# StephenNG59/ICP-symm

Hardware: AMD Instinct MI355X
Metric: icp_iterations_per_sec (higher is better)
Workload: dtype f32

## Files before the change

### icp-symm_amd/csrc/engine.cpp

```cpp
#include "engine_internal.h"
#include "robust_loss.h"
#include <limits>

void read_switches(Switches &w)
{
    auto flag = [](const char *n) { return std::getenv(n) != nullptr; };
    auto num = [](const char *n, long def) { const char *e = std::getenv(n); return e ? std::atol(e) : def; };
    auto tri = [](const char *n) { const char *e = std::getenv(n); return e ? (e[0] == '1' ? 1 : 0) : -1; };
    w.allow_any_arch = flag("SYMMICP_ALLOW_ANY_ARCH");
    w.debug_host = flag("SYMMICP_DEBUG_HOST");
    w.debug_counters = flag("SYMMICP_DEBUG_COUNTERS");
    if (const char *e = std::getenv("SYMMICP_DEBUG_TRACE")) w.debug_trace = e;
    if (const char *e = std::getenv("SYMMICP_GRID_PPC")) w.grid_ppc = std::atof(e);
    w.grid_maxlevel = (int)num("SYMMICP_GRID_MAXLEVEL", kMortonBits);
    w.grid_level = (int)num("SYMMICP_GRID_LEVEL", -1);
    if (const char *e = std::getenv("SYMMICP_FIRST_PASS")) w.first_pass = (e[0] == 'p') ? 1 : 0;
    w.oct_leaf = (int)num("SYMMICP_OCT_LEAF", 0);
    if (const char *e = std::getenv("SYMMICP_PACKET_ORDER")) w.packet_order = e[0] != '0';
    if (const char *e = std::getenv("SYMMICP_PACKET_JUMP")) w.packet_jump = (float)std::atof(e);
    w.packet_key_bits = (int)num("SYMMICP_PACKET_KEY_BITS", 16);
    w.packet_chunk = (uint32_t)num("SYMMICP_PACKET_CHUNK", 0);
    w.packet_lds_pad = (uint32_t)num("SYMMICP_PACKET_LDS_PAD", 0);
    w.packet_waves = (uint32_t)num("SYMMICP_PACKET_WAVES", 0);
    w.packet_front_cap = (uint32_t)num("SYMMICP_PACKET_FRONT_CAP", 0);
    if (const char *e = std::getenv("SYMMICP_HOOD_FRAC")) w.hood_frac = std::atof(e);
    w.no_hood = flag("SYMMICP_NO_NEIGHBOURHOOD");
    w.no_cert = flag("SYMMICP_NO_CERT");
    w.walk_full_grid = flag("SYMMICP_WALK_FULL_GRID");
    { const char *e = std::getenv("SYMMICP_HOST_LOOP"); w.host_loop = e && e[0] == '1'; }
    w.no_loop_stragglers = flag("SYMMICP_NO_LOOP_STRAGGLERS");
    w.force_comm = flag("SYMMICP_FORCE_COMM");
    if (const char *e = std::getenv("SYMMICP_PACKET_COST_KEY")) w.packet_cost_key = e[0] != '0';
    w.budget_walk = tri("SYMMICP_BUDGET_WALK");
    w.optimistic = tri("SYMMICP_OPTIMISTIC");
    w.compact = tri("SYMMICP_COMPACT");
    w.pass_blocks = (int)num("SYMMICP_PASS_BLOCKS", 2048);
    w.id_blocks = (int)num("SYMMICP_ID_BLOCKS", 2048);
    w.acc_blocks = (int)num("SYMMICP_ACC_BLOCKS", 512);
    w.fused_blocks = (int)num("SYMMICP_FUSED_BLOCKS", 512);
    w.compact_blocks = (int)num("SYMMICP_COMPACT_BLOCKS", 1280);
    w.feature_nn_splits = (int)num("SYMMICP_FEATURE_NN_SPLITS", 0);
    w.feature_nn_queries = (int)num("SYMMICP_FEATURE_NN_QUERIES", 0);
    w.tune.wave_mode_max = (uint32_t)num("SYMMICP_WAVE_MODE_MAX", 20000);
    w.tune.cells_chunk = (uint32_t)num("SYMMICP_CELLS_CHUNK", 16);
    w.tune.cells_queries = (uint32_t)num("SYMMICP_CELLS_QUERIES", 0);
    w.tune.walk_budget = (uint32_t)num("SYMMICP_WALK_BUDGET", 160);
}

void arena_begin(Arena &a, size_t want)
{
    a.off = 0;
    if (a.cap >= want) return;
    if (a.base) hipFree(a.base);
    a.base = nullptr; a.cap = 0;
    const size_t cap = want + want / 4;
    if (hipMalloc((void **)&a.base, cap) == hipSuccess) a.cap = cap;
    else (void)hipGetLastError();
}


extern "C" {

int symmicp_version(void) { return 100; }

void symmicp_config_default(symmicp_config *cfg)
{
    if (!cfg) return;
    std::memset(cfg, 0, sizeof(*cfg));
    cfg->struct_size = (int32_t)sizeof(*cfg);
    cfg->device = -1;
    cfg->mode = SYMMICP_MODE_QUIRKS;
    cfg->corr = SYMMICP_CORR_IDENTITY;
    cfg->apply = SYMMICP_APPLY_DEFAULT;
    cfg->max_iters = 10;
    cfg->diff_threshold = 1.0f;
    cfg->max_corr_dist = 0.f;
    cfg->fixed_iters = 0;
    cfg->sort_source = 1;
    cfg->verbose = 0;
    cfg->min_normal_dot = -2.0f;
    cfg->eps_rotation = 0.f;
    cfg->eps_translation = 0.f;
}

static int check_cfg(const symmicp_config *cfg)
{
    if (!cfg || cfg->struct_size != (int32_t)sizeof(symmicp_config)) return SYMMICP_ERR_ARG;
    if (!mode_known(cfg->mode)) return SYMMICP_ERR_ARG;
    if (cfg->corr < SYMMICP_CORR_IDENTITY || cfg->corr > SYMMICP_CORR_TREE) return SYMMICP_ERR_ARG;
    if (cfg->apply < SYMMICP_APPLY_DEFAULT || cfg->apply > SYMMICP_APPLY_CUMULATIVE) return SYMMICP_ERR_ARG;
    if (cfg->max_iters < 0) return SYMMICP_ERR_ARG;
    return SYMMICP_OK;
}

int symmicp_create(const symmicp_config *cfg, symmicp_ctx **out)
{
    if (!out) return SYMMICP_ERR_ARG;
    *out = nullptr;
// ... 417 lines not shown
    HIP_TRY(c, kt.alloc_temp(c->arena, n));
    HIP_TRY(c, vt.alloc_temp(c->arena, n));
    HIP_TRY(c, ws.alloc_temp(c->arena, wse));
    launch_bbox(cl.x, cl.y, cl.z, n, bbox.p, c->stream);
    uint32_t hb[6];
    HIP_TRY(c, hipMemcpyAsync(hb, bbox.p, sizeof(hb), hipMemcpyDeviceToHost, c->stream));
    HIP_TRY(c, hipStreamSynchronize(c->stream));
    float lo[3], hi[3];
    for (int k = 0; k < 3; k++) { lo[k] = ord2f(hb[k]); hi[k] = ord2f(hb[3 + k]); }
    float emax = 0.f;
    for (int k = 0; k < 3; k++) {
        if (!std::isfinite(lo[k]) || !std::isfinite(hi[k])) return fail(c, SYMMICP_ERR_ARG, "cloud has non-finite coordinates");
        emax = std::fmax(emax, hi[k] - lo[k]);
    }
    if (!(emax > 0.f)) emax = 1.f;
    const float h0 = emax * 1.00001f / (float)(1 << kMortonBits);
    launch_morton(cl.x, cl.y, cl.z, n, lo[0], lo[1], lo[2], 1.0f / h0, keys.p, vals.p, c->stream);
    radix_sort_pairs(keys.p, vals.p, kt.p, vt.p, n, 3 * kMortonBits, ws.p, wse, c->stream);
    HIP_TRY(c, hipStreamSynchronize(c->stream));
    HIP_TRY(c, hipGetLastError());
    for (int k = 0; k < 3; k++) origin[k] = lo[k];
    *h0_out = h0;
    return SYMMICP_OK;
}

static int build_octree(symmicp_ctx *c, const uint32_t *keys, const float4 *tq, uint32_t n, uint32_t leaf_max, float4 **onodes_out, TargetIndex *ix)
{
    constexpr int NL = kMortonBits + 1;
    DevBuf<uint32_t> nid;
    DevBuf<uint32_t> scan_ws, first;
    float4 *nodes = nullptr;
    HIP_TRY(c, nid.alloc_temp(c->arena, (size_t)NL * n));
    HIP_TRY(c, scan_ws.alloc_temp(c->arena, (size_t)n / 2048 + 2));
    for (int l = 0; l < NL; l++) {
        launch_oct_flags(keys, n, l, nid.p + (size_t)l * n, c->stream);
        launch_exclusive_scan(nid.p + (size_t)l * n, n, scan_ws.p, c->stream);
    }
    uint32_t last_excl[NL], kl[2] = {0, 0};
    for (int l = 0; l < NL; l++)
        HIP_TRY(c, hipMemcpyAsync(&last_excl[l], nid.p + (size_t)l * n + (n - 1), sizeof(uint32_t), hipMemcpyDeviceToHost, c->stream));
    if (n >= 2) HIP_TRY(c, hipMemcpyAsync(kl, keys + (n - 2), 2 * sizeof(uint32_t), hipMemcpyDeviceToHost, c->stream));
    HIP_TRY(c, hipStreamSynchronize(c->stream));
    uint32_t cnt[NL];
    size_t total = 0;
    for (int l = 0; l < NL; l++) {
        const int shift = 3 * (kMortonBits - l);
        const bool last_starts = (n == 1) || (shift < 30 && (kl[1] >> shift) != (kl[0] >> shift));
        cnt[l] = last_excl[l] + (last_starts ? 1u : 0u);
        ix->olevel_off[l] = (uint32_t)total;
        total += cnt[l];
    }
    ix->olevel_off[NL] = (uint32_t)total;
    for (int l = 0; l < NL; l++)
        if (cnt[l] > kOctCfMask) return fail(c, SYMMICP_ERR_SIZE, "octree level exceeds 2^28 nodes (target cloud too large for SYMMICP_CORR_TREE)");
    HIP_TRY(c, first.alloc_temp(c->arena, total + 1));
    HIP_TRY(c, keep_alloc(c, (void **)&nodes, sizeof(float4) * 2 * total));
    for (int l = 0; l < NL; l++)
        launch_oct_first(keys, n, l, nid.p + (size_t)l * n, first.p + ix->olevel_off[l], c->stream);
    for (int l = NL - 1; l >= 0; l--) {
        const bool bottom = (l == NL - 1);
        launch_oct_nodes(l, tq, n, first.p + ix->olevel_off[l], cnt[l], bottom ? nullptr : nid.p + (size_t)(l + 1) * n,
                         bottom ? 0u : cnt[l + 1], bottom ? nullptr : nodes + 2 * (size_t)ix->olevel_off[l + 1],
                         nodes + 2 * (size_t)ix->olevel_off[l], leaf_max, c->stream);
    }
    HIP_TRY(c, hipStreamSynchronize(c->stream));
    HIP_TRY(c, hipGetLastError());
    *onodes_out = nodes;
    ix->onodes = *onodes_out;
    return SYMMICP_OK;
}

static int build_index(symmicp_ctx *c, const CloudSoA &cl, uint32_t n, bool want_grid, float4 *tq, float4 *tn,
                       float4 **boxes_out, uint2 **cells_out, TargetIndex *ix_out, int32_t *glevel_out, int32_t *nlevels_out,
                       float4 **onodes_out = nullptr, uint32_t **ctop_out = nullptr, IndexNotes *notes = nullptr)
{
    DevBuf<uint32_t> order, keys;
    float origin[3], h0;
    int st = morton_order(c, cl, n, order, &keys, origin, &h0);
    if (st != SYMMICP_OK) return st;
    if (notes) { *notes = IndexNotes{}; for (int k = 0; k < 3; k++) notes->origin[k] = origin[k]; notes->h0 = h0; }
    launch_gather_f4(cl.x, cl.y, cl.z, cl.nx, cl.ny, cl.nz, order.p, n, tq, tn, c->stream);
    TargetIndex ix{};
    ix.tq = tq; ix.tn = tn; ix.n = n;
    int glevel = 0;
    if (want_grid) {
        DevBuf<uint32_t> hist;
        HIP_TRY(c, hist.alloc_temp(c->arena, 16));
        launch_level_hist(keys.p, n, hist.p, c->stream);
        uint32_t hh[16];
        HIP_TRY(c, hipMemcpyAsync(hh, hist.p, sizeof(hh), hipMemcpyDeviceToHost, c->stream));
        HIP_TRY(c, hipStreamSynchronize(c->stream));
        if (notes) std::memcpy(notes->hist, hh, sizeof(hh));
        const double ppc = c->sw.grid_ppc;
        int lcap = c->sw.grid_maxlevel;
        if (lcap > kMortonBits) lcap = kMortonBits;
        glevel = 1;
        double occ = 1.0;
        for (int l = 1; l <= lcap; l++) {
            occ += (double)hh[l];
            if ((double)n / occ >= ppc) glevel = l;
        }
        if (c->sw.grid_level >= 0) glevel = c->sw.grid_level;
        if (glevel > lcap) glevel = lcap;
        if (glevel < 0) glevel = 0;
        {
            double occ_l[kMortonBits + 1];
            double o = 1.0;
            occ_l[0] = 1.0;
            for (int l = 1; l <= kMortonBits; l++) { o += (double)hh[l]; occ_l[l] = o; }
            const int lg = glevel >= 2 ? glevel - 1 : 1;
            const double growth = occ_l[lg] / occ_l[lg - 1];
            c->target_surface_like = growth < 5.5;
            if (c->sw.first_pass >= 0) c->target_surface_like = c->sw.first_pass == 1;
        }
    }
    ix.glevel = glevel;
    if (glevel > 0) {
        const int ltop = glevel > 3 ? glevel - 3 : 0;
        const size_t ntop = (size_t)1 << (3 * ltop);
        DevBuf<uint32_t> nid_top, scan_ws;
        HIP_TRY(c, nid_top.alloc_temp(c->arena, n));
        HIP_TRY(c, scan_ws.alloc_temp(c->arena, (size_t)n / 2048 + 2));
        launch_oct_flags(keys.p, n, ltop, nid_top.p, c->stream);
        launch_exclusive_scan(nid_top.p, n, scan_ws.p, c->stream);
        uint32_t last_excl = 0, kl[2] = {0, 0};
        HIP_TRY(c, hipMemcpyAsync(&last_excl, nid_top.p + (n - 1), sizeof(uint32_t), hipMemcpyDeviceToHost, c->stream));
        if (n >= 2) HIP_TRY(c, hipMemcpyAsync(kl, keys.p + (n - 2), 2 * sizeof(uint32_t), hipMemcpyDeviceToHost, c->stream));
        HIP_TRY(c, hipStreamSynchronize(c->stream));
        const int tshift = 3 * (kMortonBits - ltop);
        const bool last_starts = (n == 1) || (tshift < 30 && (kl[1] >> tshift) != (kl[0] >> tshift));
        const size_t nblocks = (size_t)last_excl + (last_starts ? 1 : 0);
        if (notes) { notes->nblocks = (uint32_t)nblocks; notes->ctop_len = (uint32_t)ntop; }
        HIP_TRY(c, keep_alloc(c, (void **)ctop_out, sizeof(uint32_t) * ntop));
        HIP_TRY(c, hipMemsetAsync(*ctop_out, 0xFF, sizeof(uint32_t) * ntop, c->stream));
        HIP_TRY(c, keep_alloc(c, (void **)cells_out, sizeof(uint2) * nblocks * 512));
        HIP_TRY(c, hipMemsetAsync(*cells_out, 0, sizeof(uint2) * nblocks * 512, c->stream));
        launch_cell_table(keys.p, n, glevel, nid_top.p, *ctop_out, *cells_out, c->stream);
        HIP_TRY(c, hipStreamSynchronize(c->stream));
        ix.ctop = *ctop_out;
        ix.cells = *cells_out;
        ix.gdim = 1 << glevel;
        ix.ox = origin[0]; ix.oy = origin[1]; ix.oz = origin[2];
        ix.h = h0 * (float)(1 << (kMortonBits - glevel));
        ix.inv_h = (1.0f / h0) / (float)(1 << (kMortonBits - glevel));
    }
    uint32_t cnt[kMaxTreeLevels], pad[kMaxTreeLevels];
    int nl = 0;
    uint32_t m = (n + kLeaf - 1) / kLeaf;
    size_t total = 0;
    while (true) {
        cnt[nl] = m;
        pad[nl] = (m <= (uint32_t)kFan) ? m : ((m + kFan - 1) / kFan) * kFan;
        ix.level_off[nl] = (uint32_t)total;
        total += pad[nl];
        nl++;
        if (m <= (uint32_t)kFan) break;
        m = pad[nl - 1] / kFan;
        if (nl >= kMaxTreeLevels) return fail(c, SYMMICP_ERR_SIZE, "tree too deep");
    }
    ix.top = nl - 1;
    ix.ntop = cnt[nl - 1];
    HIP_TRY(c, keep_alloc(c, (void **)boxes_out, sizeof(float4) * 2 * total));
    float4 *boxes = *boxes_out;
    launch_leaf_boxes(tq, n, boxes + 2 * (size_t)ix.level_off[0], pad[0], c->stream);
    for (int l = 1; l < nl; l++)
        launch_node_boxes(boxes + 2 * (size_t)ix.level_off[l - 1], pad[l - 1], boxes + 2 * (size_t)ix.level_off[l], pad[l], c->stream);
    ix.boxes = boxes;
    HIP_TRY(c, hipStreamSynchronize(c->stream));
    HIP_TRY(c, hipGetLastError());
    if (onodes_out) {
        uint32_t leaf_max = c->target_surface_like ? 24u : 8u;
        if (c->sw.oct_leaf > 0) leaf_max = (uint32_t)c->sw.oct_leaf;
        if (notes) notes->leaf_max = leaf_max;
        st = build_octree(c, keys.p, tq, n, leaf_max, onodes_out, &ix);
        if (st != SYMMICP_OK) return st;
    }
    *ix_out = ix;
    if (glevel_out) *glevel_out = glevel;
    if (nlevels_out) *nlevels_out = nl;
    return SYMMICP_OK;
}

int symmicp_set_target(symmicp_ctx *c, const float *xyz, size_t xr, size_t xc, const float *nrm, size_t nr, size_t nc, size_t n)
{
    if (!c) return SYMMICP_ERR_ARG;
    if (!xyz || !nrm) return fail(c, SYMMICP_ERR_ARG, "null target cloud (myicp.cpp:102 assert)");
    if (n == 0 || n > 0x7fffffffull) return fail(c, SYMMICP_ERR_SIZE, "target size out of range");
    HIP_TRY(c, hipSetDevice(c->device));
    const double t0 = now_s();
    free_target(c);
    c->begun = false;
    {
        const size_t want = n * 160 + ((size_t)16 << 20);
        if (c->keep.cap < want) {
            hipFree(c->keep.base);
            c->keep = Arena{};
            if (hipMalloc((void **)&c->keep.base, want + want / 8) == hipSuccess) c->keep.cap = want + want / 8;
            else (void)hipGetLastError();
        }
    }
    arena_begin(c->arena, n * (96 + 4 * (xr + nr)) + ((size_t)1 << 20));
    double cen[3];
    DevBuf<float> tblock;
    int st = upload_planar(c, xyz, xr, xc, nrm, nr, nc, n, tblock, false, cen);
    if (st != SYMMICP_OK) return st;
    c->tgt_block = tblock.release();
    soa_from_block(c->tgt_block, n, c->tgt);
    c->n_t = (uint32_t)n;
    for (int k = 0; k < 3; k++) c->pivot[k] = (float)cen[k];
    c->st.upload_ms += (now_s() - t0) * 1e3;
    if (c->cfg.corr == SYMMICP_CORR_IDENTITY) return SYMMICP_OK;

    const double t1 = now_s();
    HIP_TRY(c, keep_alloc(c, (void **)&c->tq, sizeof(float4) * (n + 8)));
    HIP_TRY(c, hipMemsetAsync(c->tq + n, 0, sizeof(float4) * 8, c->stream));
    HIP_TRY(c, keep_alloc(c, (void **)&c->tn, sizeof(float4) * 2 * n));
    if (c->cfg.corr == SYMMICP_CORR_BRUTE) {
        launch_iota_f4(c->tgt.x, c->tgt.y, c->tgt.z, c->tgt.nx, c->tgt.ny, c->tgt.nz, c->n_t, c->tq, c->tn, c->stream);
        HIP_TRY(c, hipStreamSynchronize(c->stream));
        c->st.build_ms = (now_s() - t1) * 1e3;
        return SYMMICP_OK;
    }
    st = build_index(c, c->tgt, c->n_t, true, c->tq, c->tn, &c->boxes, &c->cells, &c->ix, &c->st.grid_level, &c->st.tree_levels,
                     &c->onodes, &c->ctop, &c->notes);
    if (st != SYMMICP_OK) { free_target(c); return st; }
    if (c->sw.debug_counters) {
        HIP_TRY(c, hipMalloc((void **)&c->dbg, 12 * sizeof(unsigned long long)));
        HIP_TRY(c, hipMemset(c->dbg, 0, 12 * sizeof(unsigned long long)));
        c->ix.dbg = c->dbg;
    }
    if (!c->sw.debug_trace.empty()) {
        HIP_TRY(c, hipMalloc((void **)&c->dbg_trace, ((size_t)1 << 22) * 8));
        HIP_TRY(c, hipMemset(c->dbg_trace, 0, ((size_t)1 << 22) * 8));
        c->ix.dbg_trace = c->dbg_trace;
    }
    c->have_index = true;
    c->st.build_ms = (now_s() - t1) * 1e3;
    return SYMMICP_OK;
}

int symmicp_set_source(symmicp_ctx *c, const float *xyz, size_t xr, size_t xc, const float *nrm, size_t nr, size_t nc, size_t n)
{
    if (!c) return SYMMICP_ERR_ARG;
    if (!xyz) return fail(c, SYMMICP_ERR_ARG, "null source cloud (myicp.cpp:102 assert)");
    if (!nrm && c->cfg.mode != SYMMICP_MODE_PLANE) return fail(c, SYMMICP_ERR_ARG, "null source normals (only SYMMICP_MODE_PLANE runs without them)");
    if (!nrm && c->cfg.min_normal_dot > -1.0f) return fail(c, SYMMICP_ERR_ARG, "min_normal_dot needs source normals");
    if (!nrm) nr = nc = 0;
    if (n == 0 || n > 0x7fffffffull) return fail(c, SYMMICP_ERR_SIZE, "source size out of range");
    HIP_TRY(c, hipSetDevice(c->device));
    const double t0 = now_s();
    forget_source(c);
    c->begun = false;
    c->trim_valid = false;
    c->rej_valid = c->rej_new = false;
    size_t b0 = 0, bc = 0;
    symmicp_shard_range(n, c->nranks, c->rank, &b0, &bc);
    const size_t nu = bc > 0 ? bc : 1;
    const size_t r0 = bc > 0 ? b0 : 0;
    arena_begin(c->arena, nu * (56 + 4 * (xr + nr)) + ((size_t)1 << 20));
    DevBuf<float> full;
    int st = upload_planar(c, xyz + r0 * xr, xr, xc, nrm ? nrm + r0 * nr : nullptr, nr, nc, nu, full, true, nullptr);
    if (st != SYMMICP_OK) return st;
    c->src_no_normals = !nrm;
    CloudSoA fs;
    soa_from_block(full.p, nu, fs);
    const uint32_t nl = bc > 0 ? (uint32_t)bc : 1;
    const bool sorted = c->cfg.corr != SYMMICP_CORR_IDENTITY && c->cfg.sort_source;
    const bool tree = c->cfg.corr == SYMMICP_CORR_TREE, brute = c->cfg.corr == SYMMICP_CORR_BRUTE;
    const uint32_t cap = shard_capacity(nl);
    const size_t per_list = (size_t)kShards * cap, ncount = (size_t)kShards * kShardStride;
    size_t off = 0;
    auto take = [&](size_t bytes) { const size_t o = off; off += (bytes + 255) & ~(size_t)255; return o; };
    const size_t o_src0 = take(sizeof(float) * 6 * nl), o_cur = take(sizeof(float) * 6 * nl);
    const size_t o_order = sorted ? take(sizeof(uint32_t) * nl) : 0;
    const size_t o_pos = take(sizeof(int32_t) * nl), o_d2 = take(sizeof(float) * nl);
    const size_t o_best = brute ? take(sizeof(unsigned long long) * nl) : 0;
    const size_t o_cert = tree ? take(sizeof(float) * 4 * nl) : 0;
    const size_t o_certk = tree ? take(sizeof(uint32_t) * 8 * nl) : 0, o_hoodr = tree ? take(sizeof(float) * 2 * nl) : 0;
    const size_t o_pkt = tree ? take(sizeof(uint32_t) * 2 * 8 * ((nl + 63) / 64)) : 0;
    const size_t o_prec = tree ? take(sizeof(float4) * 2 * nl) : 0;
    const size_t o_wl = tree ? take(sizeof(uint32_t) * 2 * per_list) : 0, o_cnt = tree ? take(sizeof(uint32_t) * 2 * ncount) : 0;
    if (off > c->src_all_cap) {
        hipFree(c->src_all);
        c->src_all = nullptr; c->src_all_cap = 0;
// ... 715 lines not shown
```

### icp-symm_amd/csrc/engine_debug.cpp

```cpp
#include "engine_internal.h"

static constexpr size_t kTraceWords = (size_t)1 << 22;
void dump_packet_trace(symmicp_ctx *c)
{
    if (FILE *f = std::fopen(c->sw.debug_trace.c_str(), "wb")) {
        std::vector<unsigned long long> t(kTraceWords);
        hipMemcpy(t.data(), c->dbg_trace, t.size() * 8, hipMemcpyDeviceToHost);
        std::fwrite(t.data(), 8, t.size(), f);
        std::fclose(f);
    }
    hipMemset(c->dbg_trace, 0, kTraceWords * 8);
}


void print_pass_counters(symmicp_ctx *c, bool first, long long list_len)
{
        unsigned long long h[12];
        hipMemcpy(h, c->ix.dbg, sizeof(h), hipMemcpyDeviceToHost);
        hipMemset(c->ix.dbg, 0, sizeof(h));
        if (first && c->cfg.corr == SYMMICP_CORR_TREE && c->target_surface_like)
            std::fprintf(stderr, "[symmicp dbg] pass %lld (packets): steps=%llu nodes+leaf candidates=%llu leaf candidates rejected=%llu points=%llu tie rescans=%llu overflows=%llu lanes wanting a scanned leaf (sum)=%llu | packet ticks (10 ns): sum=%llu max=%llu\n",
                         (long long)c->st.passes, h[0], h[4], h[5], h[3], h[2], h[1], h[8], h[7], h[6]);
        else
        std::fprintf(stderr, "[symmicp dbg] pass %lld: cells: certified=%llu (by neighbourhood %llu) scans=%llu (neighbourhoods kept %llu, not kept %llu) probes=%llu to-walk=%llu items=%llu points=%llu | walk list=%lld visits=%llu wave-max*64=%llu\n",
                     (long long)c->st.passes, h[1], h[8], h[2], h[9], h[10], h[6], h[7], h[0], h[3], list_len, h[4], h[5]);
}
```

### icp-symm_amd/csrc/engine_internal.h

```cpp
#pragma once
#include <hip/hip_runtime.h>
#include <dlfcn.h>
#include <fcntl.h>
#include <sys/mman.h>
#include <sys/stat.h>
#include <unistd.h>
#include <algorithm>
#include <chrono>
#include <cmath>
#include <cstdio>
#include <cstdlib>
#include <cstring>
#include <mutex>
#include <string>
#include <vector>

#include "symmicp.h"
#include "symmicp_internal.h"
#include "host_solve.h"


namespace symmicp {}
using namespace symmicp;

typedef struct { char internal[128]; } rcclUniqueId;
typedef void *rcclComm_t;
typedef int (*fn_ncclGetUniqueId)(rcclUniqueId *);
typedef int (*fn_ncclCommInitRank)(rcclComm_t *, int, rcclUniqueId, int);
typedef int (*fn_ncclCommDestroy)(rcclComm_t);
typedef int (*fn_ncclAllReduce)(const void *, void *, size_t, int, int, rcclComm_t, hipStream_t);
typedef const char *(*fn_ncclGetErrorString)(int);
constexpr int kNcclFloat64 = 8;
constexpr int kNcclSum = 0;

struct Rccl {
    void *handle = nullptr;
    fn_ncclGetUniqueId GetUniqueId = nullptr;
    fn_ncclCommInitRank CommInitRank = nullptr;
    fn_ncclCommDestroy CommDestroy = nullptr;
    fn_ncclAllReduce AllReduce = nullptr;
    fn_ncclGetErrorString GetErrorString = nullptr;
    std::string err;
    std::mutex mu;
    bool load()
    {
        std::lock_guard<std::mutex> lock(mu);
        if (handle && AllReduce) return true;
        const char *names[] = {"librccl.so.1", "librccl.so"};
        for (const char *nm : names) { handle = dlopen(nm, RTLD_NOW | RTLD_NOLOAD | RTLD_GLOBAL); if (handle) break; }
        if (!handle)
            for (const char *nm : names) { handle = dlopen(nm, RTLD_NOW | RTLD_GLOBAL); if (handle) break; }
        if (!handle) { err = std::string("cannot load librccl: ") + dlerror(); return false; }
        GetUniqueId = (fn_ncclGetUniqueId)dlsym(handle, "ncclGetUniqueId");
        CommInitRank = (fn_ncclCommInitRank)dlsym(handle, "ncclCommInitRank");
        CommDestroy = (fn_ncclCommDestroy)dlsym(handle, "ncclCommDestroy");
        AllReduce = (fn_ncclAllReduce)dlsym(handle, "ncclAllReduce");
        GetErrorString = (fn_ncclGetErrorString)dlsym(handle, "ncclGetErrorString");
        if (!GetUniqueId || !CommInitRank || !CommDestroy || !AllReduce) { err = "librccl misses nccl* symbols"; return false; }
        return true;
    }
};
extern Rccl g_rccl;

inline double now_s()
{
    return std::chrono::duration<double>(std::chrono::steady_clock::now().time_since_epoch()).count();
}

struct Switches {
    bool allow_any_arch = false, debug_host = false, debug_counters = false;
    std::string debug_trace;
    double grid_ppc = 3.0;
    int grid_maxlevel = kMortonBits, grid_level = -1;
    int first_pass = -1;
    int oct_leaf = 0;
    bool packet_order = true;
    bool packet_cost_key = true;
    float packet_jump = -1.0f;
    int packet_key_bits = 16;
    uint32_t packet_chunk = 0, packet_lds_pad = 0, packet_waves = 0, packet_front_cap = 0;
    double hood_frac = 0.8;
    bool no_hood = false, no_cert = false, walk_full_grid = false, host_loop = false, no_loop_stragglers = false, force_comm = false;
    int budget_walk = -1, optimistic = -1, compact = -1;
    int pass_blocks = 2048, id_blocks = 2048, acc_blocks = 512, fused_blocks = 512, compact_blocks = 1280;
    int feature_nn_splits = 0, feature_nn_queries = 0;
    PassTuning tune;
};

void read_switches(Switches &w);

struct Arena {
    char *base = nullptr;
    size_t cap = 0, off = 0;
};

struct ShmSlot {
    volatile unsigned long long seq;
    double s[SYMMICP_NSUM];
    char pad[512 - 8 - 8 * SYMMICP_NSUM];
};
static_assert(sizeof(ShmSlot) == 512, "slot = 4 cache lines");
struct ShmExchange {
    ShmSlot *slots = nullptr;
    size_t bytes = 0;
    unsigned long long count = 0;
    std::string name;
    bool owner = false;
};

struct IndexNotes {
    float origin[3] = {0, 0, 0}, h0 = 0.f;
    uint32_t hist[16] = {};
    uint32_t leaf_max = 0;
    uint32_t nblocks = 0, ctop_len = 0;
};

struct symmicp_ctx {
    Switches sw;
    Arena arena;
    Arena keep;
    std::vector<void *> keep_extra;
    ShmExchange shm;
    symmicp_config cfg{};
    int loss = SYMMICP_LOSS_NONE;
    float loss_scale = 0.f;
    float gicp_eps = 1e-3f;
    float color_lam = 0.968f;
    float4 *tgt_color = nullptr;
    float *src_int = nullptr;
    size_t tgt_color_cap = 0, src_int_cap = 0;
    bool have_tgt_color = false, have_src_int = false;
    float trim_frac = 1.0f;
    uint32_t *trim_keys = nullptr, *trim_ws = nullptr;
    size_t trim_keys_cap = 0;
    bool trim_valid = false;
    uint32_t trim_nc = 0, trim_kept = 0, trim_tau = 0;
    bool one_to_one = false;
    float med_factor = 0.0f;
    unsigned long long *uniq_table = nullptr;
    size_t uniq_table_cap = 0;
    bool rej_valid = false, rej_new = false;
    uint32_t rej_gated = 0, rej_unique = 0;
    int device = 0;
    hipStream_t stream = nullptr;
    std::string err;
    int nranks = 1, rank = 0;
    rcclComm_t comm = nullptr;
    bool external_exchange = false;
    bool sums_exchanged = false;
    uint32_t n_t = 0;
    float *tgt_block = nullptr;
    CloudSoA tgt{};
    float4 *tq = nullptr, *tn = nullptr;
    float4 *boxes = nullptr;
    float4 *onodes = nullptr;
    uint2 *cells = nullptr;
    uint32_t *ctop = nullptr;
    unsigned long long *dbg = nullptr;
    unsigned long long *dbg_trace = nullptr;
    TargetIndex ix{};
    bool have_index = false;
    bool target_surface_like = false;
    IndexNotes notes;
    float pivot[3] = {0, 0, 0};
    uint32_t n_s_total = 0, n_loc = 0, src_off = 0;
    bool src_no_normals = false;
    char *src_all = nullptr;
    size_t src_all_cap = 0;
    float *src0_block = nullptr, *cur_block = nullptr;
    CloudSoA src0{}, cur{};
    uint32_t *src_order = nullptr;
    int32_t *pos = nullptr;
    float *d2 = nullptr;
    float4 *pairrec = nullptr;
    float *cert = nullptr;
    uint32_t *certk = nullptr;
    float *hoodr = nullptr;
    uint32_t *pkt_tab = nullptr;
    uint32_t pkt_count = 0;
    bool pkt_cost_keyed = false;
    uint32_t *pkt_fallbacks = nullptr;
    unsigned long long *best64 = nullptr;
    uint32_t *worklist = nullptr, *wl_count = nullptr;
    WorkLists wl{};
    int pass_blocks = 0;
    double *partials = nullptr, *d_sums = nullptr, *h_sums = nullptr, *h_sums_dev = nullptr;
    uint32_t *ticket = nullptr;
    long long last_list_len = -1;
    long long last_uncertified = -1;
    static constexpr int kRing = 65;
    LoopState *d_loop = nullptr, *h_loop = nullptr, *h_loop_dev = nullptr;
    LoopRecord *h_ring = nullptr, *h_ring_dev = nullptr;
    unsigned long long *h_done = nullptr, *h_done_dev = nullptr;
    unsigned long long batch_seq = 0;
    bool loop_log_on = false;
    std::vector<symmicp_loop_log_entry> loop_log;
    int loop_log_batches = 0;
// ... 81 lines not shown
```

### icp-symm_amd/csrc/engine_probe.cpp

```cpp
#include "engine_internal.h"

namespace {

int copy_back(symmicp_ctx *c, void *dst, const void *src, size_t bytes)
{
    if (!dst || !bytes) return SYMMICP_OK;
    if (!src) return fail(c, SYMMICP_ERR_STATE, "probe: the context does not hold this array");
    HIP_TRY(c, hipMemcpyAsync(dst, src, bytes, hipMemcpyDeviceToHost, c->stream));
    return SYMMICP_OK;
}

bool has_target_index(const symmicp_ctx *c) { return c->have_index && c->cfg.corr == SYMMICP_CORR_TREE && c->tq && c->boxes && c->onodes; }

void fill_info(const symmicp_ctx *c, symmicp_index_info *o)
{
    const TargetIndex &ix = c->ix;
    std::memset(o, 0, sizeof(*o));
    o->struct_size = (int32_t)sizeof(*o);
    o->n = ix.n;
    o->grid_level = ix.glevel;
    o->gdim = ix.gdim;
    for (int k = 0; k < 3; k++) o->origin[k] = c->notes.origin[k];
    o->h0 = c->notes.h0;
    o->h = ix.h;
    o->inv_h = ix.inv_h;
    o->tree_levels = ix.top + 1;
    o->top = ix.top;
    o->ntop = ix.ntop;
    static_assert(sizeof(o->level_off) == sizeof(ix.level_off) && sizeof(o->olevel_off) == sizeof(ix.olevel_off), "info mirrors TargetIndex");
    std::memcpy(o->level_off, ix.level_off, sizeof(o->level_off));
    o->n_boxes = ix.level_off[ix.top] + ix.ntop;
    std::memcpy(o->olevel_off, ix.olevel_off, sizeof(o->olevel_off));
    o->n_onodes = ix.olevel_off[kMortonBits + 1];
    o->n_blocks = c->notes.nblocks;
    o->ctop_len = c->notes.ctop_len;
    o->leaf_max = c->notes.leaf_max;
    o->surface_like = c->target_surface_like ? 1 : 0;
    std::memcpy(o->level_hist, c->notes.hist, sizeof(o->level_hist));
}

}

extern "C" {

int symmicp_ctx_index_info(symmicp_ctx *c, symmicp_index_info *info)
{
    if (!c) return SYMMICP_ERR_ARG;
    if (!info || info->struct_size != (int32_t)sizeof(symmicp_index_info)) return fail(c, SYMMICP_ERR_ARG, "index_info: null info or wrong struct_size");
    if (!has_target_index(c)) return fail(c, SYMMICP_ERR_STATE, "index_info: no target index (SYMMICP_CORR_TREE after set_target)");
    fill_info(c, info);
    return SYMMICP_OK;
}

int symmicp_ctx_index_arrays(symmicp_ctx *c, float *tq, float *tn, float *boxes, uint32_t *ctop, uint32_t *cells, float *onodes)
{
    if (!c) return SYMMICP_ERR_ARG;
    if (!has_target_index(c)) return fail(c, SYMMICP_ERR_STATE, "index_arrays: no target index (SYMMICP_CORR_TREE after set_target)");
    symmicp_index_info o;
    fill_info(c, &o);
    HIP_TRY(c, hipSetDevice(c->device));
    const size_t f4 = sizeof(float4);
    const struct { void *dst; const void *src; size_t bytes; } parts[] = {
        {tq, c->tq, f4 * o.n},
        {tn, c->tn, f4 * 2 * o.n},
        {boxes, c->boxes, f4 * 2 * o.n_boxes},
        {ctop, c->ctop, sizeof(uint32_t) * (o.grid_level > 0 ? o.ctop_len : 0)},
        {cells, c->cells, sizeof(uint2) * 512 * (size_t)(o.grid_level > 0 ? o.n_blocks : 0)},
        {onodes, c->onodes, f4 * 2 * o.n_onodes},
    };
    for (const auto &p : parts) {
        const int st = copy_back(c, p.dst, p.src, p.bytes);
        if (st != SYMMICP_OK) { (void)hipStreamSynchronize(c->stream); return st; }
    }
    HIP_TRY(c, hipStreamSynchronize(c->stream));
    return SYMMICP_OK;
}

int symmicp_ctx_source_share(symmicp_ctx *c, size_t *n_local, size_t *pkt_count, int32_t *sorted, int32_t *cost_keyed, uint32_t *order,
                             uint32_t *pkt_tab)
{
    if (!c) return SYMMICP_ERR_ARG;
    if (!c->src0_block) return fail(c, SYMMICP_ERR_STATE, "source_share: no source (set_source first)");
    if (order && !c->src_order) return fail(c, SYMMICP_ERR_STATE, "source_share: the share is not sorted (it is in the caller's order)");
    if (n_local) *n_local = c->n_loc;
    if (pkt_count) *pkt_count = c->pkt_tab ? c->pkt_count : 0;
    if (sorted) *sorted = c->src_order ? 1 : 0;
    if (cost_keyed) *cost_keyed = (c->pkt_tab && c->pkt_cost_keyed) ? 1 : 0;
    if (!order && !pkt_tab) return SYMMICP_OK;
    HIP_TRY(c, hipSetDevice(c->device));
    int st = copy_back(c, order, c->src_order, sizeof(uint32_t) * c->n_loc);
    if (st == SYMMICP_OK && c->pkt_tab) st = copy_back(c, pkt_tab, c->pkt_tab, sizeof(uint32_t) * 2 * c->pkt_count);
    const hipError_t e = hipStreamSynchronize(c->stream);
    if (st != SYMMICP_OK) return st;
    HIP_TRY(c, e);
    return SYMMICP_OK;
}

int symmicp_ctx_radix_sort_probe(symmicp_ctx *c, uint32_t *keys, uint32_t *vals, size_t n, int key_bits)
{
    if (!c) return SYMMICP_ERR_ARG;
    if (key_bits < 0 || key_bits > 32 || n > 0x7fffffffull || (n && (!keys || !vals))) return fail(c, SYMMICP_ERR_ARG, "radix_sort_probe: bad arguments");
    if (n == 0) return SYMMICP_OK;
    HIP_TRY(c, hipSetDevice(c->device));
    const uint32_t m = (uint32_t)n;
    const size_t wse = radix_sort_ws_elems(m), bytes = sizeof(uint32_t) * n;
    arena_begin(c->arena, 4 * (bytes + 256) + sizeof(uint32_t) * wse + 4096);
    DevBuf<uint32_t> k, v, kt, vt, ws;
    HIP_TRY(c, k.alloc_temp(c->arena, n));
    HIP_TRY(c, v.alloc_temp(c->arena, n));
    HIP_TRY(c, kt.alloc_temp(c->arena, n));
    HIP_TRY(c, vt.alloc_temp(c->arena, n));
    HIP_TRY(c, ws.alloc_temp(c->arena, wse));
    HIP_TRY(c, hipMemcpyAsync(k.p, keys, bytes, hipMemcpyHostToDevice, c->stream));
    HIP_TRY(c, hipMemcpyAsync(v.p, vals, bytes, hipMemcpyHostToDevice, c->stream));
    HIP_TRY(c, hipStreamSynchronize(c->stream));
    radix_sort_pairs(k.p, v.p, kt.p, vt.p, m, key_bits, ws.p, wse, c->stream);
    HIP_TRY(c, hipGetLastError());
    HIP_TRY(c, hipMemcpyAsync(keys, k.p, bytes, hipMemcpyDeviceToHost, c->stream));
    HIP_TRY(c, hipMemcpyAsync(vals, v.p, bytes, hipMemcpyDeviceToHost, c->stream));
    HIP_TRY(c, hipStreamSynchronize(c->stream));
    return SYMMICP_OK;
}

int symmicp_ctx_select_probe(symmicp_ctx *c, const uint32_t *keys, size_t n, uint64_t k, uint32_t *kth_out, uint64_t *n_le_out)
{
    if (!c) return SYMMICP_ERR_ARG;
    if (!keys || !kth_out || !n_le_out || n == 0 || n > 0x7fffffffull || k < 1 || k > n) return fail(c, SYMMICP_ERR_ARG, "select_probe: bad arguments");
    HIP_TRY(c, hipSetDevice(c->device));
    const size_t bytes = sizeof(uint32_t) * n;
    arena_begin(c->arena, bytes + sizeof(uint32_t) * kTrimWsWords + 4096);
    DevBuf<uint32_t> d, ws;
    HIP_TRY(c, d.alloc_temp(c->arena, n));
    HIP_TRY(c, ws.alloc_temp(c->arena, kTrimWsWords));
    HIP_TRY(c, hipMemcpyAsync(d.p, keys, bytes, hipMemcpyHostToDevice, c->stream));
    HIP_TRY(c, hipStreamSynchronize(c->stream));
    launch_select_probe(d.p, (uint32_t)n, (uint32_t)k, ws.p, c->stream);
    HIP_TRY(c, hipGetLastError());
    uint32_t state[8] = {};
    HIP_TRY(c, hipMemcpyAsync(state, ws.p, sizeof(state), hipMemcpyDeviceToHost, c->stream));
    HIP_TRY(c, hipStreamSynchronize(c->stream));
    *kth_out = state[kTrimTauWord];
    *n_le_out = state[4];
    return SYMMICP_OK;
}

int symmicp_ctx_unique_probe(symmicp_ctx *c, const int32_t *tgt_row, const uint32_t *d2_bits, size_t n, size_t n_t, uint8_t *winner_out)
{
    if (!c) return SYMMICP_ERR_ARG;
    if (!tgt_row || !d2_bits || !winner_out || n == 0 || n > 0x7fffffffull || n_t == 0 || n_t > 0x7fffffffull) return fail(c, SYMMICP_ERR_ARG, "unique_probe: bad arguments");
    HIP_TRY(c, hipSetDevice(c->device));
    arena_begin(c->arena, (sizeof(int32_t) + sizeof(uint32_t) + 1) * n + sizeof(unsigned long long) * n_t + 4096);
    DevBuf<int32_t> d_row;
    DevBuf<uint32_t> d_d2;
    DevBuf<unsigned long long> table;
    DevBuf<uint8_t> d_win;
    HIP_TRY(c, table.alloc_temp(c->arena, n_t));
    HIP_TRY(c, d_row.alloc_temp(c->arena, n));
    HIP_TRY(c, d_d2.alloc_temp(c->arena, n));
    HIP_TRY(c, d_win.alloc_temp(c->arena, n));
    HIP_TRY(c, hipMemcpyAsync(d_row.p, tgt_row, sizeof(int32_t) * n, hipMemcpyHostToDevice, c->stream));
// ... 31 lines not shown
```

### icp-symm_amd/csrc/kernels_build.hip

```cpp
#include <cstdlib>
#include "symmicp_internal.h"
#pragma clang fp contract(off)

namespace symmicp {

__device__ __forceinline__ uint32_t f2ord(float f)
{
    uint32_t u = __float_as_uint(f);
    return (u & 0x80000000u) ? ~u : (u | 0x80000000u);
}

__global__ __launch_bounds__(256) void k_bbox(const float *__restrict__ x, const float *__restrict__ y,
                                              const float *__restrict__ z, uint32_t n, uint32_t *bbox)
{
    const float inf = __int_as_float(0x7f800000);
    float lo[3] = {inf, inf, inf}, hi[3] = {-inf, -inf, -inf};
    for (uint32_t i = blockIdx.x * blockDim.x + threadIdx.x; i < n; i += gridDim.x * blockDim.x) {
        float v[3] = {x[i], y[i], z[i]};
#pragma unroll
        for (int k = 0; k < 3; k++) {
            if (!(fabsf(v[k]) < inf)) { lo[k] = -inf; hi[k] = inf; }
            lo[k] = fminf(lo[k], v[k]); hi[k] = fmaxf(hi[k], v[k]);
        }
    }
// ... 170 lines not shown

__global__ __launch_bounds__(256) void k_deinterleave3(const float *__restrict__ raw, size_t row_stride, size_t offset, uint32_t n,
                                                       float *__restrict__ x, float *__restrict__ y, float *__restrict__ z)
{
    const uint32_t i = blockIdx.x * blockDim.x + threadIdx.x;
    if (i >= n) return;
    const float *r = raw + (size_t)i * row_stride + offset;
    x[i] = r[0]; y[i] = r[1]; z[i] = r[2];
}

void launch_deinterleave3(const float *raw, size_t row_stride, size_t offset, uint32_t n, float *x, float *y, float *z, hipStream_t s)
{
    hipLaunchKernelGGL(k_deinterleave3, dim3((n + 255) / 256), dim3(256), 0, s, raw, row_stride, offset, n, x, y, z);
}

__global__ __launch_bounds__(256) void k_gather_soa(CloudSoA src, const uint32_t *__restrict__ order, uint32_t n, CloudSoA dst)
{
    uint32_t i = blockIdx.x * blockDim.x + threadIdx.x;
    if (i >= n) return;
    uint32_t j = order[i];
    dst.x[i] = src.x[j]; dst.y[i] = src.y[j]; dst.z[i] = src.z[j];
    dst.nx[i] = src.nx[j]; dst.ny[i] = src.ny[j]; dst.nz[i] = src.nz[j];
}

__global__ __launch_bounds__(256) void k_unpermute(CloudSoA cur, const uint32_t *__restrict__ order, uint32_t n,
                                                   float *xyz, float *nrm)
{
    uint32_t i = blockIdx.x * blockDim.x + threadIdx.x;
    if (i >= n) return;
    uint32_t r = order ? order[i] : i;
    if (xyz) { xyz[3 * (size_t)r] = cur.x[i]; xyz[3 * (size_t)r + 1] = cur.y[i]; xyz[3 * (size_t)r + 2] = cur.z[i]; }
    if (nrm) { nrm[3 * (size_t)r] = cur.nx[i]; nrm[3 * (size_t)r + 1] = cur.ny[i]; nrm[3 * (size_t)r + 2] = cur.nz[i]; }
}

__global__ __launch_bounds__(256) void k_corr_out(const int32_t *__restrict__ pos, const unsigned long long *__restrict__ best64,
                                                  const float *__restrict__ d2, const float4 *__restrict__ tq,
                                                  const uint32_t *__restrict__ src_order, uint32_t n, int mode,
                                                  uint32_t tgt_offset, int32_t *idx_out, float *d2_out,
                                                  const uint32_t *__restrict__ trim_keys, uint32_t trim_tau)
{
    uint32_t i = blockIdx.x * blockDim.x + threadIdx.x;
    if (i >= n) return;
    uint32_t r = src_order ? src_order[i] : i;
    int32_t row = -1;
    if (mode == 0) row = (int32_t)(tgt_offset + i);
    else if (mode == 1) { unsigned long long b = best64[i]; row = (b == ~0ull) ? -1 : (int32_t)(uint32_t)(b & 0xFFFFFFFFull); }
    else { int32_t p = pos[i]; row = (p < 0) ? -1 : __float_as_int(tq[p].w); }
    if (trim_keys && trim_keys[i] > trim_tau) row = -1;
    if (idx_out) idx_out[r] = row;
    if (d2_out) d2_out[r] = d2 ? d2[i] : 0.0f;
}

__global__ __launch_bounds__(256) void k_level_hist(const uint32_t *__restrict__ keys, uint32_t n, uint32_t *hist16)
{
    __shared__ uint32_t h[16];
    if (threadIdx.x < 16) h[threadIdx.x] = 0;
    __syncthreads();
    for (uint32_t i = blockIdx.x * blockDim.x + threadIdx.x + 1; i < n; i += gridDim.x * blockDim.x) {
        uint32_t x = keys[i] ^ keys[i - 1];
        if (x) {
            int b = 31 - __clz((int)x);
            int lvl = kMortonBits - b / 3;
            atomicAdd(&h[lvl], 1u);
        }
    }
    __syncthreads();
    if (threadIdx.x < 16 && h[threadIdx.x]) atomicAdd(hist16 + threadIdx.x, h[threadIdx.x]);
}

__global__ __launch_bounds__(256) void k_cell_table(const uint32_t *__restrict__ keys, uint32_t n, int shift, int top_shift,
                                                    const uint32_t *__restrict__ nid_top, uint32_t *ctop, uint2 *cells)
{
    uint32_t i = blockIdx.x * blockDim.x + threadIdx.x;
    if (i >= n) return;
    const uint32_t c = keys[i] >> shift;
    const bool top_start = i == 0 || (top_shift < 30 && (keys[i - 1] >> top_shift) != (keys[i] >> top_shift));
    const uint32_t block = nid_top[i] - (top_start ? 0u : 1u);
    if (top_start) ctop[top_shift < 30 ? (keys[i] >> top_shift) : 0u] = block;
    uint2 *slot = cells + (size_t)block * 512u + (c & 511u);
    if (i == 0 || (keys[i - 1] >> shift) != c) slot->x = i;
    if (i == n - 1 || (keys[i + 1] >> shift) != c) slot->y = i + 1;
}

__global__ __launch_bounds__(256) void k_leaf_boxes(const float4 *__restrict__ tq, uint32_t n, float4 *boxes, uint32_t nleaf_padded)
{
    uint32_t l = blockIdx.x * blockDim.x + threadIdx.x;
    if (l >= nleaf_padded) return;
    const float inf = __int_as_float(0x7f800000);
    float4 lo = make_float4(inf, inf, inf, 0.f), hi = make_float4(-inf, -inf, -inf, 0.f);
    uint32_t j0 = l * kLeaf;
    for (uint32_t j = j0; j < j0 + kLeaf && j < n; j++) {
        float4 q = tq[j];
        lo.x = fminf(lo.x, q.x); lo.y = fminf(lo.y, q.y); lo.z = fminf(lo.z, q.z);
        hi.x = fmaxf(hi.x, q.x); hi.y = fmaxf(hi.y, q.y); hi.z = fmaxf(hi.z, q.z);
    }
    boxes[2 * (size_t)l] = lo; boxes[2 * (size_t)l + 1] = hi;
}

__global__ __launch_bounds__(256) void k_node_boxes(const float4 *__restrict__ child, uint32_t nchild_padded, float4 *parent,
                                                    uint32_t nparent_padded)
{
    uint32_t p = blockIdx.x * blockDim.x + threadIdx.x;
    if (p >= nparent_padded) return;
    const float inf = __int_as_float(0x7f800000);
    float4 lo = make_float4(inf, inf, inf, 0.f), hi = make_float4(-inf, -inf, -inf, 0.f);
    for (uint32_t c = p * kFan; c < p * kFan + kFan && c < nchild_padded; c++) {
        float4 a = child[2 * (size_t)c], b = child[2 * (size_t)c + 1];
        lo.x = fminf(lo.x, a.x); lo.y = fminf(lo.y, a.y); lo.z = fminf(lo.z, a.z);
        hi.x = fmaxf(hi.x, b.x); hi.y = fmaxf(hi.y, b.y); hi.z = fmaxf(hi.z, b.z);
    }
    parent[2 * (size_t)p] = lo; parent[2 * (size_t)p + 1] = hi;
}


__device__ __forceinline__ bool oct_is_start(const uint32_t *__restrict__ keys, uint32_t i, int shift)
{
    return i == 0 || (shift < 30 && (keys[i] >> shift) != (keys[i - 1] >> shift));
}

__global__ __launch_bounds__(256) void k_oct_flags(const uint32_t *__restrict__ keys, uint32_t n, int shift, uint32_t *nid)
{
    const uint32_t i = blockIdx.x * blockDim.x + threadIdx.x;
    if (i < n) nid[i] = oct_is_start(keys, i, shift) ? 1u : 0u;
}

__global__ __launch_bounds__(256) void k_oct_first(const uint32_t *__restrict__ keys, uint32_t n, int shift,
                                                   const uint32_t *__restrict__ nid, uint32_t *first)
{
    const uint32_t i = blockIdx.x * blockDim.x + threadIdx.x;
    if (i < n && oct_is_start(keys, i, shift)) first[nid[i]] = i;
}

__global__ __launch_bounds__(256) void k_oct_nodes(int level, const float4 *__restrict__ tq, uint32_t n,
                                                   const uint32_t *__restrict__ first, uint32_t n_nodes,
                                                   const uint32_t *__restrict__ nid_next, uint32_t n_nodes_next,
                                                   const float4 *__restrict__ nodes_next, float4 *nodes, uint32_t kOctLeafMax)
{
    const uint32_t id = blockIdx.x * blockDim.x + threadIdx.x;
    if (id >= n_nodes) return;
    const float inf = __int_as_float(0x7f800000);
    const uint32_t p0 = first[id], p1 = (id + 1 < n_nodes) ? first[id + 1] : n;
    const uint32_t npts = p1 - p0;
    float4 lo = make_float4(inf, inf, inf, 0.f), hi = make_float4(-inf, -inf, -inf, 0.f);
    uint32_t packed;
    if (level == kMortonBits || npts <= kOctLeafMax) {
        for (uint32_t j = p0; j < p1; j++) {
            const float4 q = tq[j];
            lo.x = fminf(lo.x, q.x); lo.y = fminf(lo.y, q.y); lo.z = fminf(lo.z, q.z);
            hi.x = fmaxf(hi.x, q.x); hi.y = fmaxf(hi.y, q.y); hi.z = fmaxf(hi.z, q.z);
        }
        packed = npts & kOctCfMask;
    } else {
        const uint32_t c0 = nid_next[p0];
        const uint32_t c1 = (id + 1 < n_nodes) ? nid_next[p1] : n_nodes_next;
        for (uint32_t c = c0; c < c1; c++) {
            const float4 a = nodes_next[2 * (size_t)c], b = nodes_next[2 * (size_t)c + 1];
            lo.x = fminf(lo.x, a.x); lo.y = fminf(lo.y, a.y); lo.z = fminf(lo.z, a.z);
            hi.x = fmaxf(hi.x, b.x); hi.y = fmaxf(hi.y, b.y); hi.z = fmaxf(hi.z, b.z);
        }
        packed = (c0 & kOctCfMask) | ((c1 - c0) << 28);
    }
    lo.w = __int_as_float((int)p0);
    hi.w = __int_as_float((int)packed);
    nodes[2 * (size_t)id] = lo;
    nodes[2 * (size_t)id + 1] = hi;
}
// ... 56 lines not shown
    hipLaunchKernelGGL(k_oct_first, dim3((n + 255) / 256), dim3(256), 0, s, keys, n, 3 * (kMortonBits - level), nid, first);
}

void launch_oct_nodes(int level, const float4 *tq, uint32_t n, const uint32_t *first, uint32_t n_nodes, const uint32_t *nid_next,
                      uint32_t n_nodes_next, const float4 *nodes_next, float4 *nodes, uint32_t leaf_max, hipStream_t s)
{
    hipLaunchKernelGGL(k_oct_nodes, dim3((n_nodes + 255) / 256), dim3(256), 0, s, level, tq, n, first, n_nodes, nid_next, n_nodes_next,
                       nodes_next, nodes, leaf_max);
}

static inline uint32_t nblk(uint32_t n, uint32_t t) { return (n + t - 1) / t; }

void launch_bbox(const float *x, const float *y, const float *z, uint32_t n, uint32_t *bbox_ord6, hipStream_t s)
{
    hipMemsetAsync(bbox_ord6, 0xFF, 3 * sizeof(uint32_t), s);
    hipMemsetAsync(bbox_ord6 + 3, 0x00, 3 * sizeof(uint32_t), s);
    uint32_t blocks = nblk(n, 256);
    if (blocks > 512) blocks = 512;
    hipLaunchKernelGGL(k_bbox, dim3(blocks), dim3(256), 0, s, x, y, z, n, bbox_ord6);
}

void launch_morton(const float *x, const float *y, const float *z, uint32_t n, float ox, float oy, float oz,
                   float inv_h0, uint32_t *keys, uint32_t *vals, hipStream_t s)
{
    hipLaunchKernelGGL(k_morton, dim3(nblk(n, 256)), dim3(256), 0, s, x, y, z, n, ox, oy, oz, inv_h0, keys, vals);
}

void launch_gather_f4(const float *x, const float *y, const float *z, const float *nx, const float *ny, const float *nz,
                      const uint32_t *order, uint32_t n, float4 *tq, float4 *tn, hipStream_t s)
{
    hipLaunchKernelGGL(k_gather_f4, dim3(nblk(n, 256)), dim3(256), 0, s, x, y, z, nx, ny, nz, order, n, tq, tn);
}

void launch_iota_f4(const float *x, const float *y, const float *z, const float *nx, const float *ny, const float *nz,
                    uint32_t n, float4 *tq, float4 *tn, hipStream_t s)
{
    hipLaunchKernelGGL(k_gather_f4, dim3(nblk(n, 256)), dim3(256), 0, s, x, y, z, nx, ny, nz, (const uint32_t *)nullptr, n, tq, tn);
}

__global__ __launch_bounds__(256) void k_offset_u32(const uint32_t *__restrict__ in, uint32_t off, uint32_t n, uint32_t *__restrict__ out)
{
    const uint32_t i = blockIdx.x * blockDim.x + threadIdx.x;
    if (i < n) out[i] = in[i] + off;
}

void launch_offset_u32(const uint32_t *in, uint32_t off, uint32_t n, uint32_t *out, hipStream_t s)
{
    hipLaunchKernelGGL(k_offset_u32, dim3(nblk(n, 256)), dim3(256), 0, s, in, off, n, out);
}

void launch_gather_soa(const CloudSoA &src, const uint32_t *order, uint32_t n, CloudSoA dst, hipStream_t s)
{
    hipLaunchKernelGGL(k_gather_soa, dim3(nblk(n, 256)), dim3(256), 0, s, src, order, n, dst);
}

void launch_unpermute(const CloudSoA &cur, const uint32_t *order, uint32_t n, float *xyz_aos, float *nrm_aos, hipStream_t s)
{
    hipLaunchKernelGGL(k_unpermute, dim3(nblk(n, 256)), dim3(256), 0, s, cur, order, n, xyz_aos, nrm_aos);
}

void launch_corr_out(const int32_t *pos, const unsigned long long *best64, const float *d2, const float4 *tq,
                     const uint32_t *src_order, uint32_t n, int mode, uint32_t tgt_offset, int32_t *idx_out, float *d2_out,
                     const uint32_t *trim_keys, uint32_t trim_tau, hipStream_t s)
{
    hipLaunchKernelGGL(k_corr_out, dim3(nblk(n, 256)), dim3(256), 0, s, pos, best64, d2, tq, src_order, n, mode, tgt_offset,
                       idx_out, d2_out, trim_keys, trim_tau);
}

void launch_level_hist(const uint32_t *keys, uint32_t n, uint32_t *hist16, hipStream_t s)
{
    hipMemsetAsync(hist16, 0, 16 * sizeof(uint32_t), s);
    uint32_t blocks = nblk(n, 256);
    if (blocks > 1024) blocks = 1024;
    hipLaunchKernelGGL(k_level_hist, dim3(blocks), dim3(256), 0, s, keys, n, hist16);
}

void launch_cell_table(const uint32_t *keys, uint32_t n, int glevel, const uint32_t *nid_top, uint32_t *ctop, uint2 *cells, hipStream_t s)
{
    const int shift = 3 * (kMortonBits - glevel);
    const int ltop = glevel > 3 ? glevel - 3 : 0;
    hipLaunchKernelGGL(k_cell_table, dim3(nblk(n, 256)), dim3(256), 0, s, keys, n, shift, 3 * (kMortonBits - ltop), nid_top, ctop, cells);
}

void launch_leaf_boxes(const float4 *tq, uint32_t n, float4 *boxes, uint32_t nleaf_padded, hipStream_t s)
{
    hipLaunchKernelGGL(k_leaf_boxes, dim3(nblk(nleaf_padded, 256)), dim3(256), 0, s, tq, n, boxes, nleaf_padded);
}

void launch_node_boxes(const float4 *child, uint32_t nchild_padded, float4 *parent, uint32_t nparent_padded, hipStream_t s)
{
    hipLaunchKernelGGL(k_node_boxes, dim3(nblk(nparent_padded, 256)), dim3(256), 0, s, child, nchild_padded, parent, nparent_padded);
}

}
```

### icp-symm_amd/csrc/kernels_pass.hip

```cpp
#include <cstdlib>
#include <type_traits>
#include "symmicp_internal.h"
#include "device_common.h"
#include "oct_walk.h"
#include "solve_core.h"
#include "robust_loss.h"
#pragma clang fp contract(off)

namespace symmicp {

template <int NA>
struct AccN {
    double v[NA];
};
typedef AccN<kNAcc> Acc;
template <bool W>
using AccT = AccN<W ? kNAccW : kNAcc>;

template <int NA>
__device__ __forceinline__ void acc_zero(AccN<NA> &a)
{
#pragma unroll
    for (int k = 0; k < NA; k++) a.v[k] = 0.0;
}
// ... 298 lines not shown
            *reinterpret_cast<float4 *>(qny) = *reinterpret_cast<const float4 *>(tgt.ny + j0);
            *reinterpret_cast<float4 *>(qnz) = *reinterpret_cast<const float4 *>(tgt.nz + j0);
        } else {
            x[0] = a.in.x[i0]; y[0] = a.in.y[i0]; z[0] = a.in.z[i0];
            if (need_n) { nx[0] = a.in.nx[i0]; ny[0] = a.in.ny[i0]; nz[0] = a.in.nz[i0]; }
            else nx[0] = ny[0] = nz[0] = 0.0f;
            qx[0] = tgt.x[j0]; qy[0] = tgt.y[j0]; qz[0] = tgt.z[j0];
            qnx[0] = tgt.nx[j0]; qny[0] = tgt.ny[j0]; qnz[0] = tgt.nz[j0];
        }
        float px[VEC], py[VEC], pz[VEC], npx[VEC], npy[VEC], npz[VEC], d2[VEC];
#pragma unroll
        for (int k = 0; k < VEC; k++) {
            px[k] = xf_row(a.X.m + 0, x[k], y[k], z[k], 1.0f); py[k] = xf_row(a.X.m + 4, x[k], y[k], z[k], 1.0f);
            pz[k] = xf_row(a.X.m + 8, x[k], y[k], z[k], 1.0f);
            npx[k] = xf_row(a.X.m + 0, nx[k], ny[k], nz[k], a.X.nrm_w); npy[k] = xf_row(a.X.m + 4, nx[k], ny[k], nz[k], a.X.nrm_w);
            npz[k] = xf_row(a.X.m + 8, nx[k], ny[k], nz[k], a.X.nrm_w);
            d2[k] = dist2(px[k], py[k], pz[k], qx[k], qy[k], qz[k]);
        }
        if (a.writeback) {
            if (VEC == 4) {
                *reinterpret_cast<float4 *>(a.out.x + i0) = *reinterpret_cast<float4 *>(px);
                *reinterpret_cast<float4 *>(a.out.y + i0) = *reinterpret_cast<float4 *>(py);
                *reinterpret_cast<float4 *>(a.out.z + i0) = *reinterpret_cast<float4 *>(pz);
                *reinterpret_cast<float4 *>(a.out.nx + i0) = *reinterpret_cast<float4 *>(npx);
                *reinterpret_cast<float4 *>(a.out.ny + i0) = *reinterpret_cast<float4 *>(npy);
                *reinterpret_cast<float4 *>(a.out.nz + i0) = *reinterpret_cast<float4 *>(npz);
            } else {
                a.out.x[i0] = px[0]; a.out.y[i0] = py[0]; a.out.z[i0] = pz[0];
                a.out.nx[i0] = npx[0]; a.out.ny[i0] = npy[0]; a.out.nz[i0] = npz[0];
            }
        }
        if (a.d2_out) {
            if (VEC == 4) *reinterpret_cast<float4 *>(a.d2_out + i0) = *reinterpret_cast<float4 *>(d2);
            else a.d2_out[i0] = d2[0];
        }
#pragma unroll
        for (int k = 0; k < VEC; k++) {
            if constexpr (OBJ == kObjColor) {
                const ColorPair cp = color_pair(a, i0 + k, j0 + k);
                pair_step<OBJ, T>(acc, h, nx[k], ny[k], nz[k], px[k], py[k], pz[k], make_float4(qx[k], qy[k], qz[k], 0.0f), make_float4(qnx[k], qny[k], qnz[k], 0.0f), d2[k], tau, &cp);
            } else
            pair_step<OBJ, T>(acc, h, nx[k], ny[k], nz[k], px[k], py[k], pz[k], make_float4(qx[k], qy[k], qz[k], 0.0f), make_float4(qnx[k], qny[k], qnz[k], 0.0f), d2[k], tau);
        }
    }
    acc_block_reduce_store(acc, a.partials, blockIdx.x);
}

template <bool W, int OBJ, bool T>
__global__ __launch_bounds__(kPassThreads) void k_pass_indexed(PassArgs a, const float4 *__restrict__ tn)
{
    AccT<W> acc; acc_zero(acc);
    const HotParams h = hot_params(a);
    const uint32_t tau = T ? a.trim_ws[kTrimTauWord] : 0u;
    const bool need_n = reads_src_normals<OBJ>(a.writeback, a.min_ndot);
    const uint32_t stride = gridDim.x * blockDim.x;
    for (uint32_t i = blockIdx.x * blockDim.x + threadIdx.x; i < a.n; i += stride) {
        float x = a.in.x[i], y = a.in.y[i], z = a.in.z[i];
        float nx = 0.0f, ny = 0.0f, nz = 0.0f;
        if (need_n) { nx = a.in.nx[i]; ny = a.in.ny[i]; nz = a.in.nz[i]; }
        float px = xf_row(a.X.m + 0, x, y, z, 1.0f), py = xf_row(a.X.m + 4, x, y, z, 1.0f), pz = xf_row(a.X.m + 8, x, y, z, 1.0f);
        if (a.writeback) {
            a.out.x[i] = px; a.out.y[i] = py; a.out.z[i] = pz;
            a.out.nx[i] = xf_row(a.X.m + 0, nx, ny, nz, a.X.nrm_w); a.out.ny[i] = xf_row(a.X.m + 4, nx, ny, nz, a.X.nrm_w);
            a.out.nz[i] = xf_row(a.X.m + 8, nx, ny, nz, a.X.nrm_w);
        }
        unsigned long long b = a.best64[i];
        uint32_t j = (uint32_t)(b & 0xFFFFFFFFull);
        float d2 = __uint_as_float((uint32_t)(b >> 32));
        bool ok = (b != ~0ull);
        if (a.pos_out) a.pos_out[i] = ok ? (int32_t)j : -1;
        if (a.d2_out) a.d2_out[i] = ok ? d2 : __int_as_float(0x7f800000);
        if (!ok) continue;
        if (a.max_d2 > 0.0f && d2 > a.max_d2) continue;
        if (T && a.trim_uniq && a.trim_keys[i] == 0xFFFFFFFFu) continue;
        if constexpr (OBJ == kObjColor) {
            const ColorPair cp = color_pair(a, i, j);
            pair_step<OBJ, T>(acc, h, nx, ny, nz, px, py, pz, tn[2 * (size_t)j], tn[2 * (size_t)j + 1], d2, tau, &cp);
        } else
        pair_step<OBJ, T>(acc, h, nx, ny, nz, px, py, pz, tn[2 * (size_t)j], tn[2 * (size_t)j + 1], d2, tau);
    }
    acc_block_reduce_store(acc, a.partials, blockIdx.x);
}

__device__ __forceinline__ uint2 cell_range(const TargetIndex &ix, uint32_t morton)
{
    const uint32_t blk = ix.ctop[morton >> 9];
    if (blk == 0xFFFFFFFFu) return make_uint2(0u, 0u);
    return ix.cells[(size_t)blk * 512u + (morton & 511u)];
}

__device__ __forceinline__ uint32_t spread3(uint32_t v)
{
    v &= 0x3ffu;
    v = (v | (v << 16)) & 0x030000ffu;
    v = (v | (v << 8)) & 0x0300f00fu;
    v = (v | (v << 4)) & 0x030c30c3u;
    v = (v | (v << 2)) & 0x09249249u;
    return v;
}

constexpr int kWaveFrontier = 512;

__device__ __forceinline__ float axis_gap2(float p, float origin, int c, float h, float margin)
{
    const float lo = origin + (float)c * h;
    const float g = fmaxf(fmaxf(lo - p, p - (lo + h)) - margin, 0.0f);
    return g * g;
}

#ifndef SLACK_FRAC
#define SLACK_FRAC 0.0625f
#endif
constexpr float kSlackFrac = SLACK_FRAC;
constexpr int kHoodSlots = 8;
constexpr uint32_t kHoodNone = 0xFFFFFFFFu;

__device__ __forceinline__ float cert_word(float L, bool hood)
{
    const uint32_t u = __float_as_uint(L);
    if (!(L > 0.0f)) return hood ? __uint_as_float(0xBF800001u) : 0.0f;
    return __uint_as_float(hood ? ((u - 1u) | 1u) : (u & ~1u));
}

__device__ __forceinline__ bool hood_test(const PassArgs &a, const TargetIndex &ix, uint32_t i, float px, float py, float pz, float m2,
                                          int32_t pos_a, float d2a, int32_t rowa, int32_t &pos_w, float &d2w)
{
    const uint4 w0 = a.certk[2 * (size_t)i], w1 = a.certk[2 * (size_t)i + 1];
    const float T = a.hoodr[i].x;
    const uint32_t cand[kHoodSlots] = {w0.x, w0.y, w0.z, w0.w, w1.x, w1.y, w1.z, w1.w};
    float4 q[kHoodSlots];
#pragma unroll
    for (int k = 0; k < kHoodSlots; k++) q[k] = ix.tq[min(cand[k], ix.n - 1u)];
    unsigned long long kw = ((unsigned long long)__float_as_uint(d2a) << 32) | (unsigned long long)(uint32_t)rowa;
    uint32_t sec = 0x7f800000u;
    pos_w = pos_a;
#pragma unroll
    for (int k = 0; k < kHoodSlots; k++) {
        const float d2 = dist2(px, py, pz, q[k].x, q[k].y, q[k].z);
        if (cand[k] < ix.n && cand[k] != (uint32_t)pos_a && d2 == d2) {
            const unsigned long long key = ((unsigned long long)__float_as_uint(d2) << 32) | (unsigned long long)(uint32_t)__float_as_int(q[k].w);
            if (key < kw) { sec = (uint32_t)(kw >> 32); kw = key; pos_w = (int32_t)cand[k]; }
            else sec = min(sec, __float_as_uint(d2));
        }
    }
    d2w = __uint_as_float((uint32_t)(kw >> 32));
    const float dl = __builtin_amdgcn_sqrtf(m2);
    if (!((__builtin_amdgcn_sqrtf(d2w) + dl) * 1.000002f < T)) return false;
    if (pos_w != pos_a) {
        a.pos_out[i] = pos_w;
        store_pair_record(a, ix, i, pos_w);
    }
    const float d1 = sqrtf(d2w) * 1.000001f;
    const float Tn = (T - dl * 1.000001f) * 0.999999f;
    const float L = fminf(sqrtf(__uint_as_float(sec)) * 0.999999f, Tn);
    if (Tn > d1 * 1.001f) {
        a.cert[i] = make_float4(px, py, pz, cert_word((L > d1) ? L : 0.0f, true));
        a.hoodr[i].x = Tn;
    } else if (pos_w != pos_a) {
        a.cert[i].w = cert_word(0.0f, true);
    }
    return true;
}

template <bool HOOD>
__device__ __forceinline__ void cells_tile(const PassArgs &a, const TargetIndex &ix, const WorkLists &wl, const Affine &X, const uint32_t i,
                                           const uint32_t shard, const bool from_list)
{
    __shared__ float s_px[kPassThreads], s_py[kPassThreads], s_pz[kPassThreads];
    __shared__ unsigned long long s_key[kPassThreads];
    __shared__ uint32_t s_second[kPassThreads];
    __shared__ int32_t s_pos[kPassThreads];
    __shared__ uint32_t s_cell0[kPassThreads];
    __shared__ __align__(8) uint16_t s_items[kPassThreads * 27];
    __shared__ uint32_t s_wsum[kPassThreads / 64 + 1];
    __shared__ uint32_t s_anyw[kPassThreads / 64];
    __shared__ uint32_t s_nmore;
    constexpr int kHoodLds = HOOD ? kPassThreads : 1;
    __shared__ float s_reach[kHoodLds];
    __shared__ uint32_t s_hcnt[kHoodLds];
    __shared__ uint32_t s_qi[kHoodLds];

    const int tid = threadIdx.x, lane = tid & 63, wave = tid >> 6;
    const bool active = i < a.n;
    const float inf = __int_as_float(0x7f800000);
    const uint32_t push_shard = from_list ? ((i / kPassThreads) & (uint32_t)(kShards - 1)) : shard;

    float px = 0.f, py = 0.f, pz = 0.f;
    Best b;
    b.d2 = inf; b.pos = -1; b.row = 0x7fffffff;
    uint32_t mask = 0;
    uint32_t mask_rest = 0;
    bool defer = false, searched = false, probe = false, uncert = false, hood_ok = false;
    float lim = 0.f, lim_full = 0.f;
    float reach = 0.f;
    if (active) {
        const float x = a.in.x[i], y = a.in.y[i], z = a.in.z[i];
        const int32_t prev = a.pos_prev ? a.pos_prev[i] : -1;
        float clear = 0.0f, rx = 0.0f, ry = 0.0f, rz = 0.0f;
        if (a.use_slack) { const float4 ce = a.cert[i]; rx = ce.x; ry = ce.y; rz = ce.z; clear = ce.w; }
        px = xf_row(X.m + 0, x, y, z, 1.0f); py = xf_row(X.m + 4, x, y, z, 1.0f); pz = xf_row(X.m + 8, x, y, z, 1.0f);
        if (prev >= 0 && (uint32_t)prev < ix.n) {
            const float4 q = ix.tq[prev];
            const float d2 = dist2(px, py, pz, q.x, q.y, q.z);
            const int32_t row = __float_as_int(q.w);
            if (d2 <= inf) { b.d2 = d2; b.pos = prev; b.row = row; }
        }
        bool certified = false;
        if (a.use_slack && b.pos >= 0 && !from_list) {
            const float m2 = dist2(px, py, pz, rx, ry, rz);
            certified = (__builtin_amdgcn_sqrtf(b.d2) + __builtin_amdgcn_sqrtf(m2)) * 1.000002f < clear;
            if (!certified && (__float_as_uint(clear) & 1u) && a.certk) {
                int32_t pw; float d2w;
                if (hood_test(a, ix, i, px, py, pz, m2, b.pos, b.d2, b.row, pw, d2w)) {
                    certified = hood_ok = true; b.pos = pw; b.d2 = d2w;
                }
            }
        }
        if (!certified) {
            uncert = true;
            defer = true;
            if (b.pos >= 0 && ix.glevel > 0) {
                const float margin = 2e-3f * ix.h;
                const float gmax = (float)ix.gdim;
                const float rb = __builtin_amdgcn_sqrtf(b.d2) * 1.00001f;
                lim = rb + kSlackFrac * ix.h;
                const float r = lim + margin;
                const float lx = (px - r - ix.ox) * ix.inv_h, hx = (px + r - ix.ox) * ix.inv_h;
                const float ly = (py - r - ix.oy) * ix.inv_h, hy = (py + r - ix.oy) * ix.inv_h;
                const float lz = (pz - r - ix.oz) * ix.inv_h, hz = (pz + r - ix.oz) * ix.inv_h;
                const int x0 = (int)floorf(fminf(fmaxf(lx, 0.0f), gmax - 1.0f)), x1 = (int)floorf(fminf(fmaxf(hx, 0.0f), gmax - 1.0f));
                const int y0 = (int)floorf(fminf(fmaxf(ly, 0.0f), gmax - 1.0f)), y1 = (int)floorf(fminf(fmaxf(hy, 0.0f), gmax - 1.0f));
                const int z0 = (int)floorf(fminf(fmaxf(lz, 0.0f), gmax - 1.0f)), z1 = (int)floorf(fminf(fmaxf(hz, 0.0f), gmax - 1.0f));
                const int nx = x1 - x0, ny = y1 - y0, nz = z1 - z0;
                if (nx <= 2 && ny <= 2 && nz <= 2) {
                    defer = false;
                    searched = true;
                    const float thr2 = lim * lim * 1.00001f;
                    float gx[3], gy[3], gz[3];
#pragma unroll
                    for (int k = 0; k < 3; k++) {
                        gx[k] = (k <= nx) ? axis_gap2(px, ix.ox, x0 + k, ix.h, margin) : inf;
                        gy[k] = (k <= ny) ? axis_gap2(py, ix.oy, y0 + k, ix.h, margin) : inf;
                        gz[k] = (k <= nz) ? axis_gap2(pz, ix.oz, z0 + k, ix.h, margin) : inf;
                    }
#pragma unroll
                    for (int kz = 0; kz < 3; kz++)
#pragma unroll
                        for (int ky = 0; ky < 3; ky++)
#pragma unroll
                            for (int kx = 0; kx < 3; kx++) {
                                const float g2 = (gx[kx] + gy[ky]) + gz[kz];
                                if (g2 <= thr2) mask |= 1u << (kx + 3 * ky + 9 * kz);
                            }
                    s_cell0[tid] = (uint32_t)x0 | ((uint32_t)y0 << 10) | ((uint32_t)z0 << 20);
                    reach = rb;
                }
            }
            if (defer && b.pos >= 0 && ix.glevel > 0) {
                const float fx = (px - ix.ox) * ix.inv_h, fy = (py - ix.oy) * ix.inv_h, fz = (pz - ix.oz) * ix.inv_h;
                const float gmax = (float)ix.gdim;
                if (fx >= 0.0f && fy >= 0.0f && fz >= 0.0f && fx < gmax && fy < gmax && fz < gmax) {
                    const int cx = (int)fx, cy = (int)fy, cz = (int)fz;
                    const int x0 = max(cx - 1, 0), y0 = max(cy - 1, 0), z0 = max(cz - 1, 0);
                    const int x1 = min(cx + 1, ix.gdim - 1), y1 = min(cy + 1, ix.gdim - 1), z1 = min(cz + 1, ix.gdim - 1);
                    const int ax = max(cx - ((fx - (float)cx) < 0.5f ? 1 : 0), 0), bx = min(ax + 1, ix.gdim - 1);
                    const int ay = max(cy - ((fy - (float)cy) < 0.5f ? 1 : 0), 0), by = min(ay + 1, ix.gdim - 1);
                    const int az = max(cz - ((fz - (float)cz) < 0.5f ? 1 : 0), 0), bz = min(az + 1, ix.gdim - 1);
#pragma unroll
                    for (int kz = 0; kz < 3; kz++)
#pragma unroll
                        for (int ky = 0; ky < 3; ky++)
#pragma unroll
                            for (int kx = 0; kx < 3; kx++) {
                                const int X = x0 + kx, Y = y0 + ky, Z = z0 + kz;
                                const uint32_t bit = 1u << (kx + 3 * ky + 9 * kz);
                                if (X <= x1 && Y <= y1 && Z <= z1) {
                                    if (X >= ax && X <= bx && Y >= ay && Y <= by && Z >= az && Z <= bz) mask |= bit;
                                    else mask_rest |= bit;
                                }
                            }
                    s_cell0[tid] = (uint32_t)x0 | ((uint32_t)y0 << 10) | ((uint32_t)z0 << 20);
                    float face = inf, face8 = inf;
                    if (x0 > 0) face = fminf(face, px - (ix.ox + (float)x0 * ix.h));
                    if (y0 > 0) face = fminf(face, py - (ix.oy + (float)y0 * ix.h));
                    if (z0 > 0) face = fminf(face, pz - (ix.oz + (float)z0 * ix.h));
                    if (x1 < ix.gdim - 1) face = fminf(face, (ix.ox + (float)(x1 + 1) * ix.h) - px);
                    if (y1 < ix.gdim - 1) face = fminf(face, (ix.oy + (float)(y1 + 1) * ix.h) - py);
                    if (z1 < ix.gdim - 1) face = fminf(face, (ix.oz + (float)(z1 + 1) * ix.h) - pz);
                    if (ax > 0) face8 = fminf(face8, px - (ix.ox + (float)ax * ix.h));
                    if (ay > 0) face8 = fminf(face8, py - (ix.oy + (float)ay * ix.h));
                    if (az > 0) face8 = fminf(face8, pz - (ix.oz + (float)az * ix.h));
                    if (bx < ix.gdim - 1) face8 = fminf(face8, (ix.ox + (float)(bx + 1) * ix.h) - px);
                    if (by < ix.gdim - 1) face8 = fminf(face8, (ix.oy + (float)(by + 1) * ix.h) - py);
                    if (bz < ix.gdim - 1) face8 = fminf(face8, (ix.oz + (float)(bz + 1) * ix.h) - pz);
                    lim = face8 - 2e-3f * ix.h;
                    lim_full = face - 2e-3f * ix.h;
                    probe = true;
                    defer = false;
                    reach = __builtin_amdgcn_sqrtf(b.d2) * 1.00001f;
                }
            }
            if (defer) {
                a.pos_out[i] = b.pos;
                a.d2_out[i] = b.d2;
                a.cert[i].w = 0.0f;
                a.pairrec[2 * (size_t)i + 1].w = 2.0f;
                sl_push(wl.work, push_shard, i);
            }
        }
    }
    if (!from_list) {
        const unsigned long long mu = __ballot(uncert);
        if (lane == 0 && mu) atomicAdd(wl.work.counts + shard * kShardStride + 1, (uint32_t)__popcll(mu));
    }
    s_px[tid] = px; s_py[tid] = py; s_pz[tid] = pz;
    s_pos[tid] = b.pos;
    s_key[tid] = (b.pos >= 0) ? (((unsigned long long)__float_as_uint(b.d2) << 32) | (unsigned long long)(uint32_t)b.row) : ~0ull;
    s_second[tid] = 0x7f800000u;
    if (HOOD && reach > 0.0f && a.certk) {
        const float hint = a.hoodr[i].y;
        reach = fminf(probe ? lim_full : lim, hint > 0.0f ? fmaxf(hint, 1.01f * reach) : 2.0f * reach);
    } else reach = 0.0f;
    if (HOOD) { s_reach[tid] = reach; s_hcnt[tid] = 0; s_qi[tid] = i; }
    uint32_t total = 0, total_all = 0;
    for (int round = 0; round < 2; round++) {
    const uint32_t cnt = (uint32_t)__popc(mask);
    uint32_t incl = cnt;
#pragma unroll
    for (int off = 1; off < 64; off <<= 1) {
        const uint32_t u = __shfl_up(incl, off, 64);
        if (lane >= off) incl += u;
    }
    if (lane == 63) s_wsum[wave] = incl;
    if (round == 0) {
        const unsigned long long any3 = __ballot(searched || probe);
        if (lane == 0) s_anyw[wave] = (any3 != 0ull);
    }
    __syncthreads();
    uint32_t base = 0;
    total = 0;
#pragma unroll
    for (int w = 0; w < kPassThreads / 64; w++) {
        const uint32_t ws = s_wsum[w];
        if (w < wave) base += ws;
        total += ws;
    }
    total_all += total;
    if (round == 0 && !ix.dbg) {
        uint32_t any = 0;
#pragma unroll
        for (int w = 0; w < kPassThreads / 64; w++) any |= s_anyw[w];
        if (!any) return;
    }
    {
        uint32_t slot = base + incl - cnt;
        uint32_t m = mask;
        while (m) {
            const int bit = __ffs((int)m) - 1;
            m &= m - 1;
            s_items[slot++] = (uint16_t)((tid << 5) | bit);
        }
        if (tid == 0) s_nmore = 0;
    }
    __syncthreads();
    constexpr uint32_t kItemMax = 16;
    uint2 *s_more = reinterpret_cast<uint2 *>(s_items + ((total + 3u) & ~3u));
    const uint32_t more_cap = (uint32_t)(kPassThreads * 27 - ((total + 3u) & ~3u)) / 4u;
    auto scan_merge = [&](bool have, int q, uint32_t j0, uint32_t j1) {
        unsigned long long mykey = ~0ull;
        uint32_t my2nd = 0x7f800000u;
        int32_t mypos = -1;
        if (have) {
            const float qx = s_px[q], qy = s_py[q], qz = s_pz[q];
            const float t2 = HOOD ? s_reach[q] * s_reach[q] : 0.0f;
            for (uint32_t j = j0; j < j1; j += 4) {
                float4 t4[4];
#pragma unroll
                for (int k = 0; k < 4; k++) t4[k] = ix.tq[min(j + (uint32_t)k, j1 - 1)];
#pragma unroll
                for (int k = 0; k < 4; k++) {
                    if (j + (uint32_t)k < j1) {
                        const float d2 = dist2(qx, qy, qz, t4[k].x, t4[k].y, t4[k].z);
                        if (HOOD && d2 < t2) {
                            const uint32_t hs = atomicAdd(&s_hcnt[q], 1u);
                            if (hs < (uint32_t)kHoodSlots) reinterpret_cast<uint32_t *>(a.certk)[(size_t)s_qi[q] * kHoodSlots + hs] = j + (uint32_t)k;
                        }
                        if (d2 == d2) {
                            const unsigned long long key = ((unsigned long long)__float_as_uint(d2) << 32) |
                                                           (unsigned long long)(uint32_t)__float_as_int(t4[k].w);
                            if (key < mykey) { my2nd = (uint32_t)(mykey >> 32); mykey = key; mypos = (int32_t)(j + k); }
                            else my2nd = min(my2nd, __float_as_uint(d2));
                        }
                    }
                }
            }
            if (mypos >= 0) {
                const unsigned long long old = atomicMin(&s_key[q], mykey);
                uint32_t offer;
                if (mykey < old) offer = min((uint32_t)(old >> 32), my2nd);
                else if (mykey == old) offer = my2nd;
                else offer = (uint32_t)(mykey >> 32);
                atomicMin(&s_second[q], offer);
            }
        }
        __syncthreads();
        if (mypos >= 0 && s_key[q] == mykey) s_pos[q] = mypos;
    };
    for (uint32_t it0 = 0; it0 < total; it0 += kPassThreads) {
        const uint32_t it = it0 + tid;
        int q = 0;
        uint32_t j0 = 0, j1 = 0;
        if (it < total) {
            const uint32_t item = s_items[it];
            q = (int)(item >> 5);
            const int bit = (int)(item & 31u);
            const int kz = bit / 9, ky = (bit - 9 * kz) / 3, kx = bit - 9 * kz - 3 * ky;
            const uint32_t c0 = s_cell0[q];
            const uint32_t cx = (c0 & 1023u) + (uint32_t)kx, cy = ((c0 >> 10) & 1023u) + (uint32_t)ky, cz = (c0 >> 20) + (uint32_t)kz;
            const uint2 rng = cell_range(ix, (spread3(cz) << 2) | (spread3(cy) << 1) | spread3(cx));
            if (ix.dbg) atomicAdd(ix.dbg + 3, (unsigned long long)(rng.y - rng.x));
            j0 = rng.x; j1 = rng.y;
            while (j1 > j0 && j1 - j0 > kItemMax) {
                const uint32_t js = j0 + ((j1 - j0 - 1u) / kItemMax) * kItemMax;
                const uint32_t e = atomicAdd(&s_nmore, 1u);
                if (e >= more_cap) break;
                s_more[e] = make_uint2((uint32_t)q | ((j1 - js) << 8), js);
                j1 = js;
            }
        }
        scan_merge(it < total && j1 > j0, q, j0, j1);
    }
    __syncthreads();
    {
        const uint32_t nmore = min(s_nmore, more_cap);
        for (uint32_t e0 = 0; e0 < nmore; e0 += kPassThreads) {
            const uint32_t e = e0 + tid;
            int q = 0;
            uint32_t j0 = 0, j1 = 0;
            if (e < nmore) { const uint2 m = s_more[e]; q = (int)(m.x & 255u); j0 = m.y; j1 = m.y + (m.x >> 8); }
            scan_merge(e < nmore && j1 > j0, q, j0, j1);
        }
    }
    __syncthreads();

    bool more = false;
    if (round == 0 && probe) {
        const float d1 = sqrtf(__uint_as_float((uint32_t)(s_key[tid] >> 32))) * 1.00001f;
        if (!(d1 * 1.02f < lim)) { more = (mask_rest != 0); lim = lim_full; }
    }
    mask = more ? mask_rest : 0u;
    if (round == 1) break;
    {
        const unsigned long long anym = __ballot(more);
        if (lane == 0) s_anyw[wave] = (anym != 0ull);
        __syncthreads();
        uint32_t any = 0;
#pragma unroll
        for (int w = 0; w < kPassThreads / 64; w++) any |= s_anyw[w];
        if (!any) break;
    }
    }
    if (ix.dbg) {
        if (tid == 0) atomicAdd(ix.dbg + 0, (unsigned long long)total_all);
        const unsigned long long mc = __ballot(active && !defer && !searched && !probe), ms = __ballot(searched), mp = __ballot(probe), md = __ballot(defer);
        const unsigned long long mh = __ballot(hood_ok);
        if (lane == 0) {
            atomicAdd(ix.dbg + 8, (unsigned long long)__popcll(mh));
            atomicAdd(ix.dbg + 1, (unsigned long long)__popcll(mc)); atomicAdd(ix.dbg + 2, (unsigned long long)__popcll(ms));
            atomicAdd(ix.dbg + 6, (unsigned long long)__popcll(mp)); atomicAdd(ix.dbg + 7, (unsigned long long)__popcll(md));
        }
    }

    if (active && (searched || probe)) {
        const unsigned long long key = s_key[tid];
        const float d1sq = __uint_as_float((uint32_t)(key >> 32));
        const float d1 = sqrtf(d1sq) * 1.000001f;
        a.pos_out[i] = s_pos[tid];
        a.d2_out[i] = d1sq;
        if (probe && !(d1 < lim)) {
            a.cert[i].w = 0.0f;
            a.pairrec[2 * (size_t)i + 1].w = 2.0f;
            sl_push(wl.work, push_shard, i);
        } else {
            const float second = sqrtf(__uint_as_float(s_second[tid])) * 0.999999f;
            const float L = fminf(second, lim * 0.99999f);
            bool hood = false;
            const float Tq = HOOD ? fminf(s_reach[tid], lim) : 0.0f;
            if (Tq > 0.0f) {
                const uint32_t hc = s_hcnt[tid];
                const float T = Tq * 0.99999f;
                hood = T > d1 && hc >= 1u && hc <= (uint32_t)kHoodSlots;
                if (hood) {
                    uint32_t *slots = reinterpret_cast<uint32_t *>(a.certk) + (size_t)i * kHoodSlots;
#pragma unroll
                    for (int k = 1; k < kHoodSlots; k++) if ((uint32_t)k >= hc) slots[k] = kHoodNone;
                }
                const float scale = fminf(fmaxf(__powf(6.5f / ((float)hc + 0.5f), 0.4f), 0.4f), 1.5f);
                a.hoodr[i] = make_float2(hood ? T : 0.0f, Tq * scale);
                if (ix.dbg) atomicAdd(ix.dbg + (hood ? 9 : 10), 1ull);
            }
            const float Lw = cert_word((L > d1) ? L : 0.0f, hood);
            a.cert[i] = make_float4(px, py, pz, Lw);
            store_pair_record(a, ix, i, s_pos[tid]);
        }
    }
}

template <bool HOOD>
__global__ __launch_bounds__(kPassThreads) void k_search_cells(PassArgs a, TargetIndex ix, WorkLists wl, uint32_t chunk, uint32_t qshift)
{
    const uint32_t tile = xcd_remap_chunked(blockIdx.x, chunk);
    const uint32_t i = threadIdx.x < (1u << qshift) ? (tile << qshift) + threadIdx.x : 0xFFFFFFFFu;
    cells_tile<HOOD>(a, ix, wl, a.X, i, tile & (kShards - 1), false);
}

constexpr int kFusedList = 2048;

template <typename T>
__device__ __forceinline__ T in_vgpr(T v)
{
    asm volatile("" : "+v"(v));
    return v;
}
typedef float f32x4_t __attribute__((ext_vector_type(4)));
template <typename T>
__device__ __forceinline__ __attribute__((address_space(1))) T *gcol(unsigned long long base)
{
    return (__attribute__((address_space(1))) T *)base;
}
__device__ __forceinline__ float4 as_float4(f32x4_t v) { return make_float4(v.x, v.y, v.z, v.w); }

#ifndef FUSED_WAVES
#define FUSED_WAVES 2
#endif
#ifndef COMPACT_WAVES
#define COMPACT_WAVES 5
#endif
#ifndef FUSED_PPT
#define FUSED_PPT 1u
#endif
template <bool ACC, bool W, int OBJ>
__global__ __launch_bounds__(kPassThreads, ACC ? FUSED_WAVES : COMPACT_WAVES) void k_pass_fused(PassArgs a, TargetIndex ix, WorkLists wl)
{
    static_assert(ACC || !W, "the search-only form has no sums to weight");
    static_assert(ACC || OBJ == kObjSym, "the search-only form has no rows");
    const bool need_n = reads_src_normals<OBJ>(false, a.min_ndot);
    constexpr int kList = ACC ? kFusedList : kFusedList / 2;
    __shared__ uint32_t s_list[kList];
    __shared__ uint32_t s_cnt, s_total;
    __shared__ unsigned long long s_col[ACC ? 10 : 1];
    AccT<W> acc;
    if (ACC) acc_zero(acc);
    if (threadIdx.x == 0) { s_cnt = 0; s_total = 0; }
    if (ACC && threadIdx.x == 0) {
        s_col[0] = (unsigned long long)a.in.x; s_col[1] = (unsigned long long)a.in.y; s_col[2] = (unsigned long long)a.in.z;
        s_col[3] = (unsigned long long)a.in.nx; s_col[4] = (unsigned long long)a.in.ny; s_col[5] = (unsigned long long)a.in.nz;
        s_col[6] = (unsigned long long)a.pairrec; s_col[7] = (unsigned long long)a.cert;
    }
    __syncthreads();
    int stop = 0;
    HotParams h;
    if (ACC && a.loop) {
        stop = a.loop->stop;
        const float4 *xp = reinterpret_cast<const float4 *>(&in_vgpr(a.loop)->Xapply);
        const float4 r0 = xp[0], r1 = xp[1], r2 = xp[2];
// ... 876 lines not shown
```

### icp-symm_amd/csrc/symmicp_internal.h

```cpp
#pragma once
#include <hip/hip_runtime.h>
#include <stdint.h>
#include <stddef.h>
#include "symmicp.h"

namespace symmicp {

constexpr int kNSum = SYMMICP_NSUM;
constexpr int kNAcc = 37;
constexpr int kNAccW = 38;
constexpr double kListDropped = 4294967296.0;
constexpr int kLeaf = 8;
constexpr int kFan = 8;
constexpr int kMaxTreeLevels = 12;
constexpr int kMortonBits = 10;
constexpr int kPassThreads = 256;
constexpr int kBruteTile = 1024;
constexpr int kBruteQ = 4;

constexpr bool mode_device_solves(int mode)
{
    return mode == SYMMICP_MODE_QUIRKS || mode == SYMMICP_MODE_PAPER || mode == SYMMICP_MODE_PLANE || mode == SYMMICP_MODE_GICP;
}
constexpr bool mode_known(int mode) { return mode_device_solves(mode) || mode == SYMMICP_MODE_P2P || mode == SYMMICP_MODE_COLOR; }
constexpr int mode_solves_as(int mode) { return mode == SYMMICP_MODE_COLOR ? SYMMICP_MODE_PLANE : mode; }

constexpr int kObjSym = 0, kObjPlane = 1, kObjGicp = 2, kObjColor = 3;
constexpr int mode_obj(int mode)
{
    return mode == SYMMICP_MODE_PLANE ? kObjPlane : mode == SYMMICP_MODE_GICP ? kObjGicp : mode == SYMMICP_MODE_COLOR ? kObjColor : kObjSym;
}

struct Affine {
    float m[12];
    float nrm_w;
};

struct CloudSoA {
    float *x, *y, *z, *nx, *ny, *nz;
};

struct TargetIndex {
    const float4 *tq;
    const float4 *tn;
    uint32_t n;
    const float4 *boxes;
    uint32_t level_off[kMaxTreeLevels];
    int32_t top;
    uint32_t ntop;
    const uint32_t *ctop;
    const uint2 *cells;
    int32_t glevel;
    int32_t gdim;
    float ox, oy, oz;
    float h, inv_h;
    unsigned long long *dbg;
    unsigned long long *dbg_trace;
    const float4 *onodes;
    uint32_t olevel_off[kMortonBits + 2];
};

constexpr uint32_t kOctCfMask = 0x0FFFFFFFu;
__host__ __device__ inline uint32_t oct_nch(uint32_t packed) { return packed >> 28; }
__host__ __device__ inline uint32_t oct_cf(uint32_t packed) { return packed & kOctCfMask; }

constexpr int kShards = 64;
constexpr int kShardStride = 16;
struct ShardList {
    uint32_t *items;
    uint32_t *counts;
    uint32_t cap;
};
struct WorkLists {
    ShardList work;
    ShardList retry;
};

struct LoopState {
    float X[16];
    Affine Xapply;
    int32_t stop;
    int32_t reason;
    int32_t iters;
    int32_t small_step;
};
enum { LOOP_RUNNING = 0, LOOP_DONE = 1, LOOP_REDO_PASS = 2, LOOP_HOST_SOLVE = 3, LOOP_SLOW = 4 };
struct LoopConfig {
    int32_t mode, fixed_iters, max_iters, incremental, tree;
    float diff_threshold, eps_rotation, eps_translation, nrm_w;
    float pivot[3];
    uint32_t uncertified_limit;
    int32_t walk_in_loop;
    uint32_t list_limit;
};
struct LoopRecord {
    double sums[SYMMICP_NSUM];
    float increment[16], X[16];
    float rcond;
    int32_t status;
    int32_t solved;
    int32_t pad;
    int32_t list_len, reserved;
};

struct PassArgs {
    CloudSoA in, out;
    uint32_t n;
    uint32_t tgt_offset;
    Affine X;
    float pivot[3];
    float max_d2;
    float min_ndot;
    int32_t p2p;
    int32_t writeback;
    const unsigned long long *best64;
    int32_t *pos_prev;
    float *d2_out;
    int32_t *pos_out;
    double *partials;
    float4 *pairrec;
    int32_t budget_walk;
    int32_t refresh_records;
    float4 *cert;
    uint4 *certk;
    float2 *hoodr;
    int32_t make_hood;
    int32_t use_slack;
    const LoopState *loop;
    uint32_t partial_cols, partial_col0;
    const uint2 *pkt_tab;
    uint32_t pkt_count;
    uint32_t pkt_waves;
    uint32_t pkt_front_cap;
    uint32_t *pkt_fallbacks;
    uint32_t pkt_chunk, pkt_lds_pad;
    int32_t loss;
    float loss_scale;
    int32_t obj;
    float gicp_k;
    uint32_t *trim_keys;
    uint32_t *trim_ws;
    uint32_t *trim_host;
    float trim_rho;
    unsigned long long *uniq_table;
    const uint32_t *uniq_order;
    uint32_t uniq_n_t;
    int32_t trim_uniq;
    float med_f2;
    const float4 *tgt_color;
    const float *src_int;
    float color_lam, color_om;
};
constexpr uint32_t kTrimWsWords = 16 + 3 * 2048;
constexpr uint32_t kTrimTauWord = 3;

struct PassTuning {
    uint32_t wave_mode_max = 20000u;
    uint32_t cells_chunk = 16u;
    uint32_t cells_queries = 0u;
    uint32_t walk_budget = 160u;
};

void launch_pass_identity(const PassArgs &a, CloudSoA tgt, int blocks, bool vec4_ok, hipStream_t s);
void launch_pass_indexed(const PassArgs &a, const float4 *tn , int blocks, hipStream_t s);
void launch_pass_tree_split(const PassArgs &a, const TargetIndex &ix, const WorkLists &wl, int acc_blocks, uint32_t walk_blocks,
                            int stage, int compact_blocks, const PassTuning &tune, hipStream_t s, hipEvent_t *ev);
void launch_pass_tree_first(const PassArgs &a, const TargetIndex &ix, const WorkLists &wl, int acc_blocks, hipStream_t s, hipEvent_t *ev);
uint32_t walk_blocks_full(const WorkLists &wl);
uint32_t shard_capacity(uint32_t n_points);
void launch_final_reduce(const double *partials, int blocks, double *out_dev, double *out_host_mapped, uint32_t *ticket,
                         unsigned long long seq, uint32_t *counters_to_clear, int keep_nonempty, hipStream_t s);
void launch_pass_fused(const PassArgs &a, const TargetIndex &ix, const WorkLists &wl, int blocks, hipStream_t s);
void launch_loop_stragglers(const PassArgs &a, const TargetIndex &ix, const WorkLists &wl, int list_blocks, const PassTuning &tune, hipStream_t s);
void launch_reduce_solve(const double *partials, int blocks, double *out_dev, int mode, LoopState *loop, LoopConfig cfg, LoopRecord *ring, int ring_len,
                         uint32_t *counters_to_clear, hipStream_t s);
void launch_solve_probe(int mode, int exact_rc, const symmicp_sums *sums, int n, const float *pivot, const float *X_in, int32_t *status, float *pbar,
                        float *qbar, float *a, float *t, float *rcond, float *out16, float *X_out, hipStream_t s);
void launch_loop_end(const LoopState *loop, LoopState *host_copy, unsigned long long *done_flag, unsigned long long seq, hipStream_t s);
void launch_publish(const double *sums_dev, double *out_host_mapped, unsigned long long seq, hipStream_t s);
void launch_nn_brute(const CloudSoA &src, uint32_t n_s, const Affine &X, const float4 *tq, uint32_t n_t,
                     unsigned long long *best64, hipStream_t s);

void launch_bbox(const float *x, const float *y, const float *z, uint32_t n, uint32_t *bbox_ord6, hipStream_t s);
void launch_morton(const float *x, const float *y, const float *z, uint32_t n, float ox, float oy, float oz,
                   float inv_h0, uint32_t *keys, uint32_t *vals, hipStream_t s);
void radix_sort_pairs(uint32_t *keys, uint32_t *vals, uint32_t *keys_tmp, uint32_t *vals_tmp, uint32_t n,
                      int key_bits, uint32_t *hist_ws, size_t hist_ws_elems, hipStream_t s);
size_t radix_sort_ws_elems(uint32_t n);
void launch_gather_f4(const float *x, const float *y, const float *z, const float *nx, const float *ny, const float *nz,
                      const uint32_t *order, uint32_t n, float4 *tq, float4 *tn, hipStream_t s);
void launch_gather_soa(const CloudSoA &src, const uint32_t *order, uint32_t n, CloudSoA dst, hipStream_t s);
void launch_offset_u32(const uint32_t *in, uint32_t off, uint32_t n, uint32_t *out, hipStream_t s);
void launch_packet_runs(const CloudSoA &src, uint32_t n, float jump_factor, uint2 *runs, uint32_t *keys, uint32_t *vals, uint32_t *count, int key_bits, hipStream_t s);
void launch_packet_cost(const CloudSoA &src, const uint2 *runs, uint32_t npk, const TargetIndex &ix, uint32_t *keys, int key_bits, hipStream_t s);
void launch_packet_table(const uint32_t *order, const uint2 *runs, uint32_t npk, uint2 *tab, hipStream_t s);
void launch_deinterleave3(const float *raw, size_t row_stride, size_t offset, uint32_t n, float *x, float *y, float *z, hipStream_t s);
void launch_level_hist(const uint32_t *keys, uint32_t n, uint32_t *hist16, hipStream_t s);
void launch_cell_table(const uint32_t *keys, uint32_t n, int glevel, const uint32_t *nid_top, uint32_t *ctop, uint2 *cells, hipStream_t s);
void launch_oct_flags(const uint32_t *keys, uint32_t n, int level, uint32_t *nid, hipStream_t s);
void launch_exclusive_scan(uint32_t *data, uint32_t n, uint32_t *tile_ws , hipStream_t s);
void launch_oct_first(const uint32_t *keys, uint32_t n, int level, const uint32_t *nid, uint32_t *first, hipStream_t s);
void launch_oct_nodes(int level, const float4 *tq, uint32_t n, const uint32_t *first, uint32_t n_nodes, const uint32_t *nid_next,
                      uint32_t n_nodes_next, const float4 *nodes_next, float4 *nodes, uint32_t leaf_max, hipStream_t s);
void launch_leaf_boxes(const float4 *tq, uint32_t n, float4 *boxes, uint32_t nleaf_padded, hipStream_t s);
void launch_node_boxes(const float4 *child, uint32_t nchild_padded, float4 *parent, uint32_t nparent_padded, hipStream_t s);
void launch_iota_f4(const float *x, const float *y, const float *z, const float *nx, const float *ny, const float *nz,
                    uint32_t n, float4 *tq, float4 *tn, hipStream_t s);
void launch_unpermute(const CloudSoA &cur, const uint32_t *order, uint32_t n, float *xyz_aos, float *nrm_aos, hipStream_t s);
void launch_corr_out(const int32_t *pos, const unsigned long long *best64, const float *d2, const float4 *tq,
                     const uint32_t *src_order, uint32_t n, int mode, uint32_t tgt_offset, int32_t *idx_out, float *d2_out,
                     const uint32_t *trim_keys , uint32_t trim_tau, hipStream_t s);

void launch_trim_select(const PassArgs &a, int corr, CloudSoA tgt, const float4 *tn, hipStream_t s);
void launch_select_probe(const uint32_t *keys, uint32_t n, uint32_t k, uint32_t *ws, hipStream_t s);
void launch_unique_probe(const int32_t *tgt_row, const uint32_t *d2_bits, uint32_t n, unsigned long long *table, uint32_t n_t,
                         uint8_t *winner_out, hipStream_t s);

void launch_identity_d2(const CloudSoA &in, const Affine &X, const CloudSoA &tgt, uint32_t tgt_offset, uint32_t n, float *d2, hipStream_t s);
void launch_pairs_d2(const CloudSoA &in, const Affine &X, const int32_t *pos, const float4 *tq, uint32_t n_t, uint32_t n, float *d2, hipStream_t s);
void launch_normals_knn(const TargetIndex &ix, int k, const float vp[3], float *nrm_out, float *curv_out, hipStream_t s);
void launch_knn(const TargetIndex &ix, int k, int32_t *rows_out, float *d2_out, hipStream_t s);

void launch_color_permute_target(const float *intensity, const float *grad3, const float4 *tq, uint32_t n, float4 *dst, hipStream_t s);
void launch_color_permute_source(const float *intensity, const uint32_t *order, uint32_t off, uint32_t n, float *dst, hipStream_t s);
void launch_color_unpermute_source(const float *src_int, const uint32_t *order, uint32_t n, float *out_rows, hipStream_t s);
void launch_color_gradient(const TargetIndex &ix, const float *intensity_rows, const int32_t *knn_rows, int k, float4 *rec_rows, float *grad_rows,
                           hipStream_t s);

void launch_voxel_keys(const CloudSoA &cl, uint32_t n, float inv, const int lo[3], uint64_t nx, uint64_t ny, uint32_t *keys, uint32_t *vals,
                       hipStream_t s);
void launch_voxel_segments(const uint32_t *keys, uint32_t n, uint32_t *vid_excl, uint32_t *first, uint32_t *scan_ws, uint32_t *m0_out,
                           hipStream_t s);
void launch_voxel_keep(const uint32_t *first, uint32_t m0, uint32_t min_points, uint32_t *kid_excl, uint32_t *scan_ws, uint32_t *kfirst,
                       uint32_t *kcount, uint32_t *m_out, hipStream_t s);
void launch_voxel_mean(const CloudSoA &sorted, const uint32_t *kfirst, const uint32_t *kcount, uint32_t m, int with_normals, float *xyz_out,
                       float *nrm_out, int32_t *count_out, hipStream_t s);
void launch_voxel_of(const uint32_t *keys, const uint32_t *rows, const uint32_t *vid_excl, const uint32_t *first, const uint32_t *kid_excl,
                     uint32_t n, uint32_t min_points, int32_t *voxel_of, hipStream_t s);

void launch_radius_count(const TargetIndex &ix, float r2, int32_t *count_rows, hipStream_t s);
void launch_radius_fill(const TargetIndex &ix, float r2, const uint32_t *offs_rows, int32_t *rows_out, float *d2_out, hipStream_t s);
void launch_spfh(const TargetIndex &ix, float r2, float *spfh_sorted, float *spfh_rows , int32_t *count_rows, hipStream_t s);
void launch_fpfh(const TargetIndex &ix, float r2, const float *spfh_sorted, float *fpfh_rows, hipStream_t s);


void launch_feature_nn(const float *fa, uint32_t na, const float *fb, uint32_t nb, int queries_per_thread, uint32_t splits, void *partial,
                       int32_t *nn_out, float *d2_out, float *second_out, hipStream_t s);
size_t feature_nn_partial_bytes(uint32_t na, uint32_t splits);
void launch_ransac_hyp(const float *pq8, uint32_t m, uint32_t H, unsigned long long base, float max_dist2, float edge2, float *hyp,
                       uint8_t *status, int32_t *inliers, uint32_t *surv, uint32_t *n_surv, hipStream_t s);
void launch_ransac_eval(const float *pq8, uint32_t m, const float *hyp, const uint32_t *surv, const uint32_t *n_surv, uint32_t n_surv_host,
                        float max_dist2, int32_t *inliers, hipStream_t s);
void launch_ransac_argmax(const uint8_t *status, const int32_t *inliers, uint32_t H, unsigned long long *best, hipStream_t s);

}
```

### icp-symm_amd/py/symmicp/__init__.py

```python
import ctypes as C
import os
import sys

import numpy as np

_PKG = os.path.dirname(os.path.abspath(__file__))
_ROOT = os.path.dirname(os.path.dirname(_PKG))
LIB_PATH = os.environ.get("SYMMICP_LIB") or os.path.join(_ROOT, "lib", "libsymmicp.so")

NSUM = 40
UNIQUE_ID_BYTES = 128
OK, ERR_ARG, ERR_SIZE, ERR_DEGENERATE, ERR_IO, ERR_HIP, ERR_STATE, ERR_COMM = range(8)
ERR_NO_CONSENSUS = 8
RANSAC_EVALUATED, RANSAC_REPEATED, RANSAC_EDGE, RANSAC_DEGENERATE, RANSAC_FAR = range(5)
MODE_QUIRKS, MODE_PAPER, MODE_P2P, MODE_PLANE, MODE_GICP, MODE_COLOR = 0, 1, 2, 3, 5, 7
CORR_IDENTITY, CORR_BRUTE, CORR_TREE = 0, 1, 2
APPLY_DEFAULT, APPLY_INCREMENTAL, APPLY_CUMULATIVE = 0, 1, 2
LOSS_NONE, LOSS_HUBER, LOSS_TUKEY, LOSS_CAUCHY, LOSS_GEMAN_MCCLURE = range(5)
_LOSS_NAMES = {"none": LOSS_NONE, "huber": LOSS_HUBER, "tukey": LOSS_TUKEY, "cauchy": LOSS_CAUCHY,
               "geman_mcclure": LOSS_GEMAN_MCCLURE}

_STATUS_NAMES = {0: "OK", 1: "ERR_ARG", 2: "ERR_SIZE", 3: "ERR_DEGENERATE", 4: "ERR_IO", 5: "ERR_HIP",
                 6: "ERR_STATE", 7: "ERR_COMM", 8: "ERR_NO_CONSENSUS"}


class SymmIcpError(RuntimeError):
    def __init__(self, status, msg=""):
        self.status = status
        super().__init__("symmicp: %s (%d) %s" % (_STATUS_NAMES.get(status, "?"), status, msg))


class Config(C.Structure):
    _fields_ = [("struct_size", C.c_int32), ("device", C.c_int32), ("mode", C.c_int32), ("corr", C.c_int32),
                ("apply", C.c_int32), ("max_iters", C.c_int32), ("diff_threshold", C.c_float),
                ("max_corr_dist", C.c_float), ("fixed_iters", C.c_int32), ("sort_source", C.c_int32),
                ("verbose", C.c_int32), ("min_normal_dot", C.c_float), ("eps_rotation", C.c_float),
                ("eps_translation", C.c_float), ("host_loop", C.c_int32), ("reserved", C.c_int32 * 1)]


class Sums(C.Structure):
    _fields_ = [("s", C.c_double * NSUM)]


class IterResult(C.Structure):
    _fields_ = [("status", C.c_int32), ("iter", C.c_int32), ("diff", C.c_float), ("rcond", C.c_float),
                ("pairs", C.c_double), ("increment", C.c_float * 16), ("sums", Sums)]


class Result(C.Structure):
    _fields_ = [("status", C.c_int32), ("iters", C.c_int32), ("diff_initial", C.c_float), ("diff_final", C.c_float),
                ("transform", C.c_float * 16), ("diffs", C.c_float * 64), ("seconds_total", C.c_double)]


class LoopLogEntry(C.Structure):
    _fields_ = [("sums", C.c_double * NSUM), ("increment", C.c_float * 16), ("X", C.c_float * 16), ("rcond", C.c_float),
                ("iter", C.c_int32), ("status", C.c_int32), ("solved", C.c_int32), ("list_len", C.c_int32), ("reason", C.c_int32),
                ("batch", C.c_int32), ("reserved", C.c_int32)]


LOOP_RUNNING, LOOP_DONE, LOOP_REDO_PASS, LOOP_HOST_SOLVE, LOOP_SLOW = 0, 1, 2, 3, 4


class Stats(C.Structure):
    _fields_ = [("last_pass_ms", C.c_double), ("sum_pass_ms", C.c_double), ("passes", C.c_int64),
                ("build_ms", C.c_double), ("upload_ms", C.c_double), ("grid_level", C.c_int32),
                ("tree_levels", C.c_int32), ("pass_blocks", C.c_int64), ("bytes_algorithmic_per_pass", C.c_int64),
                ("kernel_ms", C.c_double * 8), ("kernel_launches", C.c_int64 * 8), ("pass_ms_head", C.c_double * 8), ("passes_timed", C.c_int64),
                ("loop_passes", C.c_int64), ("loop_straggler_passes", C.c_int64), ("packet_fallbacks", C.c_int64),
                ("allreduce_ms", C.c_double), ("allreduce_timed", C.c_int64)]


class RansacConfig(C.Structure):
    _fields_ = [("struct_size", C.c_uint32), ("hypotheses", C.c_uint32), ("seed", C.c_uint64), ("max_dist", C.c_float),
                ("edge_ratio", C.c_float), ("refits", C.c_int32), ("reserved", C.c_int32)]


class RansacResult(C.Structure):
    _fields_ = [("best_hypothesis", C.c_int32), ("evaluated", C.c_int32), ("inliers_ransac", C.c_int32), ("inliers_final", C.c_int32),
                ("rmse_final", C.c_double), ("transform", C.c_double * 16)]


class IndexInfo(C.Structure):
    _fields_ = [("struct_size", C.c_int32), ("n", C.c_uint32), ("grid_level", C.c_int32), ("gdim", C.c_int32), ("origin", C.c_float * 3),
                ("h0", C.c_float), ("h", C.c_float), ("inv_h", C.c_float), ("tree_levels", C.c_int32), ("top", C.c_int32), ("ntop", C.c_uint32),
                ("level_off", C.c_uint32 * 12), ("n_boxes", C.c_uint32), ("olevel_off", C.c_uint32 * 12), ("n_onodes", C.c_uint32),
                ("n_blocks", C.c_uint32), ("ctop_len", C.c_uint32), ("leaf_max", C.c_uint32), ("surface_like", C.c_int32),
                ("level_hist", C.c_uint32 * 16)]


KERNEL_SLOTS = ["k_search_cells", "(gap)", "k_search_walk", "k_accumulate", "k_final_reduce", "single_pass_kernel", "whole_pass"]


EXPORTS = [
    "symmicp_config_default", "symmicp_create", "symmicp_destroy", "symmicp_last_error", "symmicp_set_config",
    "symmicp_version", "symmicp_set_source", "symmicp_set_target", "symmicp_align", "symmicp_begin", "symmicp_step",
    "symmicp_get_transform", "symmicp_format_result", "symmicp_get_pivot", "symmicp_get_correspondences", "symmicp_get_source",
    "symmicp_local_source_count", "symmicp_local_source_offset", "symmicp_get_certificates", "symmicp_solve", "symmicp_comm_get_unique_id",
    "symmicp_comm_init_rank", "symmicp_set_sums", "symmicp_comm_init_shm", "symmicp_shard_range", "symmicp_get_stats", "symmicp_reset_stats", "symmicp_enable_timing",
    "symmicp_pcd_read", "symmicp_pcd_write", "symmicp_estimate_normals", "symmicp_ctx_estimate_normals", "symmicp_ctx_knn",
    "symmicp_set_robust_loss", "symmicp_get_robust_loss", "symmicp_robust_weight", "symmicp_set_gicp_epsilon", "symmicp_get_gicp_epsilon",
    "symmicp_ctx_solve_probe", "symmicp_ctx_loop_solve", "symmicp_set_loop_log", "symmicp_get_loop_log",
    "symmicp_voxel_downsample", "symmicp_ctx_voxel_downsample",
    "symmicp_radius_search", "symmicp_ctx_radius_search", "symmicp_fpfh", "symmicp_ctx_fpfh",
    "symmicp_feature_nn", "symmicp_ctx_feature_nn", "symmicp_feature_correspondences", "symmicp_ctx_feature_correspondences",
    "symmicp_ransac_config_default", "symmicp_ransac", "symmicp_ctx_ransac", "symmicp_ctx_ransac_hypotheses",
    "symmicp_ctx_index_info", "symmicp_ctx_index_arrays", "symmicp_ctx_source_share", "symmicp_ctx_radix_sort_probe", "symmicp_ctx_scan_probe",
    "symmicp_set_trim_fraction", "symmicp_get_trim_fraction", "symmicp_get_trim_state", "symmicp_ctx_select_probe",
    "symmicp_set_one_to_one", "symmicp_get_one_to_one", "symmicp_set_median_factor", "symmicp_get_median_factor",
    "symmicp_get_rejection_state", "symmicp_ctx_unique_probe",
    "symmicp_set_color_weight", "symmicp_get_color_weight", "symmicp_set_source_intensity", "symmicp_set_target_intensity",
    "symmicp_get_source_intensity", "symmicp_intensity_gradient", "symmicp_ctx_intensity_gradient", "symmicp_pcd_read_intensity",
]

_lib = None


def _hip_runtime_first():
    if "torch" in sys.modules or os.environ.get("SYMMICP_NO_TORCH_PRELOAD"):
        return
    try:
        import torch
    except Exception:
        pass


def lib():
    global _lib
    if _lib is not None:
        return _lib
    if not os.path.exists(LIB_PATH):
        raise SymmIcpError(ERR_HIP, "libsymmicp.so not built at %s (run `make -C icp-symm_amd`); no CPU fallback" % LIB_PATH)
    _hip_runtime_first()
    L = C.CDLL(LIB_PATH, mode=C.RTLD_GLOBAL)
    fp = C.POINTER(C.c_float)
    vp = C.c_void_p
    L.symmicp_config_default.argtypes = [C.POINTER(Config)]
    L.symmicp_config_default.restype = None
    L.symmicp_create.argtypes = [C.POINTER(Config), C.POINTER(vp)]
    L.symmicp_destroy.argtypes = [vp]
    L.symmicp_destroy.restype = None
    L.symmicp_last_error.argtypes = [vp]
    L.symmicp_last_error.restype = C.c_char_p
    L.symmicp_set_config.argtypes = [vp, C.POINTER(Config)]
    for nm in ("symmicp_set_source", "symmicp_set_target"):
        getattr(L, nm).argtypes = [vp, fp, C.c_size_t, C.c_size_t, fp, C.c_size_t, C.c_size_t, C.c_size_t]
    L.symmicp_align.argtypes = [vp, fp, C.POINTER(Result)]
    L.symmicp_begin.argtypes = [vp, fp, C.POINTER(IterResult)]
    L.symmicp_step.argtypes = [vp, C.POINTER(IterResult)]
    L.symmicp_get_transform.argtypes = [vp, fp]
    L.symmicp_get_pivot.argtypes = [vp, fp]
    L.symmicp_format_result.argtypes = [fp, C.c_char_p, C.c_size_t]
    L.symmicp_format_result.restype = C.c_size_t
    L.symmicp_get_correspondences.argtypes = [vp, C.POINTER(C.c_int32), fp, C.c_size_t]
    L.symmicp_get_source.argtypes = [vp, fp, fp, C.c_size_t]
    L.symmicp_local_source_count.argtypes = [vp]
    L.symmicp_local_source_count.restype = C.c_size_t
    L.symmicp_local_source_offset.argtypes = [vp]
    L.symmicp_local_source_offset.restype = C.c_size_t
    L.symmicp_solve.argtypes = [C.c_int, C.POINTER(Sums), fp, fp, fp, fp, fp, fp, fp]
    L.symmicp_comm_get_unique_id.argtypes = [vp]
    L.symmicp_comm_init_rank.argtypes = [vp, C.c_int, C.c_int, vp]
    L.symmicp_set_sums.argtypes = [vp, C.POINTER(Sums)]
    L.symmicp_comm_init_shm.argtypes = [vp, C.c_int, C.c_int, C.c_char_p]
    L.symmicp_shard_range.argtypes = [C.c_size_t, C.c_int, C.c_int, C.POINTER(C.c_size_t), C.POINTER(C.c_size_t)]
    L.symmicp_get_stats.argtypes = [vp, C.POINTER(Stats)]
    L.symmicp_reset_stats.argtypes = [vp]
    L.symmicp_enable_timing.argtypes = [vp, C.c_int]
    L.symmicp_pcd_read.argtypes = [C.c_char_p, fp, fp, C.c_size_t, C.POINTER(C.c_int)]
    L.symmicp_pcd_read.restype = C.c_long
    L.symmicp_pcd_write.argtypes = [C.c_char_p, fp, fp, C.c_size_t, C.c_int]
    L.symmicp_estimate_normals.argtypes = [C.c_int, fp, C.c_size_t, C.c_size_t, C.c_size_t, C.c_int, fp, fp, fp]
    L.symmicp_ctx_estimate_normals.argtypes = [vp, fp, C.c_size_t, C.c_size_t, C.c_size_t, C.c_int, fp, fp, fp]
    L.symmicp_ctx_knn.argtypes = [vp, fp, C.c_size_t, C.c_size_t, C.c_size_t, C.c_int, C.POINTER(C.c_int32), fp]
    L.symmicp_set_robust_loss.argtypes = [vp, C.c_int, C.c_float]
    L.symmicp_get_robust_loss.argtypes = [vp, C.POINTER(C.c_int), C.POINTER(C.c_float)]
    L.symmicp_robust_weight.argtypes = [C.c_int, C.c_float, C.c_float]
    L.symmicp_robust_weight.restype = C.c_float
    L.symmicp_set_gicp_epsilon.argtypes = [vp, C.c_float]
    L.symmicp_get_gicp_epsilon.argtypes = [vp, C.POINTER(C.c_float)]
    i32p = C.POINTER(C.c_int32)
    L.symmicp_ctx_solve_probe.argtypes = [vp, C.c_int, C.c_int, C.POINTER(Sums), C.c_size_t, fp, fp, i32p, fp, fp, fp, fp, fp, fp, fp]
    L.symmicp_ctx_loop_solve.argtypes = [vp, C.POINTER(Sums), fp, fp, i32p, fp, i32p, fp, fp, fp, fp, fp, i32p]
    L.symmicp_set_loop_log.argtypes = [vp, C.c_int]
    L.symmicp_get_loop_log.argtypes = [vp, C.POINTER(LoopLogEntry), C.c_size_t, C.POINTER(C.c_size_t)]
    vox = [fp, C.c_size_t, C.c_size_t, fp, C.c_size_t, C.c_size_t, C.c_size_t, C.c_float, C.c_int, fp, fp, i32p, i32p, C.c_size_t,
           C.POINTER(C.c_size_t)]
    L.symmicp_voxel_downsample.argtypes = [C.c_int] + vox
    L.symmicp_ctx_voxel_downsample.argtypes = [vp] + vox
    rad = [fp, C.c_size_t, C.c_size_t, C.c_size_t, C.c_float, i32p, C.POINTER(C.c_int64), i32p, fp, C.c_size_t, C.POINTER(C.c_size_t)]
    L.symmicp_radius_search.argtypes = [C.c_int] + rad
    L.symmicp_ctx_radius_search.argtypes = [vp] + rad
    fpf = [fp, C.c_size_t, C.c_size_t, fp, C.c_size_t, C.c_size_t, C.c_size_t, C.c_float, fp, fp, i32p]
    L.symmicp_fpfh.argtypes = [C.c_int] + fpf
    L.symmicp_ctx_fpfh.argtypes = [vp] + fpf
    fnn = [fp, C.c_size_t, fp, C.c_size_t, i32p, fp, fp]
    L.symmicp_feature_nn.argtypes = [C.c_int] + fnn
    L.symmicp_ctx_feature_nn.argtypes = [vp] + fnn
    fco = [fp, C.c_size_t, fp, C.c_size_t, C.c_int, C.c_float, i32p, fp, C.c_size_t, C.POINTER(C.c_size_t)]
    L.symmicp_feature_correspondences.argtypes = [C.c_int] + fco
    L.symmicp_ctx_feature_correspondences.argtypes = [vp] + fco
    u8p = C.POINTER(C.c_uint8)
    rsc = [fp, C.c_size_t, C.c_size_t, C.c_size_t, fp, C.c_size_t, C.c_size_t, C.c_size_t, i32p, C.c_size_t, C.POINTER(RansacConfig)]
    L.symmicp_ransac_config_default.argtypes = [C.POINTER(RansacConfig)]
    L.symmicp_ransac_config_default.restype = None
    L.symmicp_ransac.argtypes = [C.c_int] + rsc + [fp, C.POINTER(RansacResult), u8p, u8p, i32p]
    L.symmicp_ctx_ransac.argtypes = [vp] + rsc + [fp, C.POINTER(RansacResult), u8p, u8p, i32p]
    L.symmicp_ctx_ransac_hypotheses.argtypes = [vp] + rsc + [fp, u8p, fp]
    u32p, szp = C.POINTER(C.c_uint32), C.POINTER(C.c_size_t)
    L.symmicp_ctx_index_info.argtypes = [vp, C.POINTER(IndexInfo)]
    L.symmicp_ctx_index_arrays.argtypes = [vp, fp, fp, fp, u32p, u32p, fp]
    L.symmicp_ctx_source_share.argtypes = [vp, szp, szp, i32p, i32p, u32p, u32p]
    L.symmicp_ctx_radix_sort_probe.argtypes = [vp, u32p, u32p, C.c_size_t, C.c_int]
    L.symmicp_ctx_scan_probe.argtypes = [vp, u32p, C.c_size_t]
    u64p = C.POINTER(C.c_uint64)
    L.symmicp_set_trim_fraction.argtypes = [vp, C.c_float]
    L.symmicp_get_trim_fraction.argtypes = [vp, fp]
    L.symmicp_get_trim_state.argtypes = [vp, u64p, u64p, fp]
    L.symmicp_set_one_to_one.argtypes = [vp, C.c_int]
    L.symmicp_get_one_to_one.argtypes = [vp, C.POINTER(C.c_int)]
    L.symmicp_set_median_factor.argtypes = [vp, C.c_float]
    L.symmicp_get_median_factor.argtypes = [vp, fp]
    L.symmicp_get_rejection_state.argtypes = [vp, u64p, u64p, u64p, fp]
    L.symmicp_ctx_unique_probe.argtypes = [vp, i32p, u32p, C.c_size_t, C.c_size_t, C.POINTER(C.c_uint8)]
    L.symmicp_ctx_select_probe.argtypes = [vp, u32p, C.c_size_t, C.c_uint64, u32p, u64p]
    L.symmicp_set_color_weight.argtypes = [vp, C.c_float]
    L.symmicp_get_color_weight.argtypes = [vp, fp]
    L.symmicp_set_source_intensity.argtypes = [vp, fp, C.c_size_t, C.c_size_t]
    L.symmicp_set_target_intensity.argtypes = [vp, fp, C.c_size_t, fp, C.c_size_t, C.c_size_t, C.c_size_t]
    L.symmicp_get_source_intensity.argtypes = [vp, fp, C.c_size_t]
    grd = [fp, C.c_size_t, C.c_size_t, fp, C.c_size_t, C.c_size_t, fp, C.c_size_t, C.c_size_t, C.c_int, fp]
    L.symmicp_intensity_gradient.argtypes = [C.c_int] + grd
    L.symmicp_ctx_intensity_gradient.argtypes = [vp] + grd
    L.symmicp_pcd_read_intensity.argtypes = [C.c_char_p, fp, C.c_size_t, C.POINTER(C.c_int)]
    L.symmicp_pcd_read_intensity.restype = C.c_long
    _lib = L
    return L


def _fptr(a):
    return a.ctypes.data_as(C.POINTER(C.c_float))


def _cloud(a):
    a = np.ascontiguousarray(a, dtype=np.float32)
    if a.ndim != 2 or a.shape[1] != 3:
        raise ValueError("cloud must be [N,3]")
    return a


def default_config(**kw):
    cfg = Config()
    lib().symmicp_config_default(C.byref(cfg))
    for k, v in kw.items():
        if not hasattr(cfg, k):
            raise AttributeError(k)
        setattr(cfg, k, v)
    return cfg


def pcd_read(path):
    L = lib()
    hn = C.c_int(0)
    n = L.symmicp_pcd_read(os.fsencode(path), None, None, 0, C.byref(hn))
    if n < 0:
        raise SymmIcpError(-n, "pcd_read(%s)" % path)
    xyz = np.zeros((n, 3), np.float32)
    nrm = np.zeros((n, 3), np.float32)
    r = L.symmicp_pcd_read(os.fsencode(path), _fptr(xyz), _fptr(nrm), n, C.byref(hn))
    if r != n:
        raise SymmIcpError(-r if r < 0 else ERR_IO, "pcd_read(%s)" % path)
    return xyz, (nrm if hn.value else None)


def pcd_read_intensity(path):
    L = lib()
    kind = C.c_int(0)
    n = L.symmicp_pcd_read_intensity(os.fsencode(path), None, 0, C.byref(kind))
    if n < 0:
        raise SymmIcpError(-n, "pcd_read_intensity(%s)" % path)
    if kind.value == 0:
        return None, 0
    out = np.zeros(n, np.float32)
    r = L.symmicp_pcd_read_intensity(os.fsencode(path), _fptr(out), n, C.byref(kind))
    if r != n:
        raise SymmIcpError(-r if r < 0 else ERR_IO, "pcd_read_intensity(%s)" % path)
    return out, kind.value


def pcd_write(path, xyz, nrm=None, binary=False):
    xyz = _cloud(xyz)
    nrm_p = None
    if nrm is not None:
        nrm = _cloud(nrm)
# ... 588 lines not shown
        hyp = np.zeros((H, 12), np.float32)
        status = np.zeros(H, np.uint8)
        piv = np.zeros(6, np.float32)
        self._chk(self._L.symmicp_ctx_ransac_hypotheses(self._h, _fptr(src), 3, 1, src.shape[0], _fptr(tgt), 3, 1, tgt.shape[0], _i32ptr(pairs),
                                                        pairs.shape[0], C.byref(cfg), _fptr(hyp), status.ctypes.data_as(C.POINTER(C.c_uint8)),
                                                        _fptr(piv)))
        return hyp, status, piv.reshape(2, 3)

    def enable_timing(self, on=True):
        self._chk(self._L.symmicp_enable_timing(self._h, int(on)))

    def reset_stats(self):
        self._chk(self._L.symmicp_reset_stats(self._h))

    def stats(self):
        s = Stats()
        self._chk(self._L.symmicp_get_stats(self._h, C.byref(s)))
        d = {k: getattr(s, k) for k, _ in Stats._fields_}
        d["kernel_ms"] = list(s.kernel_ms)
        d["kernel_launches"] = list(s.kernel_launches)
        d["pass_ms_head"] = list(s.pass_ms_head)
        return d

    def solve_probe(self, mode, sums, exact_rc, pivot=None, X_in=None):
        S = np.ascontiguousarray(np.asarray(sums, np.float64).reshape(-1, NSUM))
        n = S.shape[0]
        o = dict(status=np.zeros(n, np.int32), pbar=np.zeros((n, 3), np.float32), qbar=np.zeros((n, 3), np.float32),
                 a=np.zeros((n, 3), np.float32), t=np.zeros((n, 3), np.float32), rcond=np.zeros(n, np.float32),
                 out16=np.zeros((n, 4, 4), np.float32))
        pv = None if pivot is None else _fptr(np.ascontiguousarray(pivot, np.float32))
        xin = xout = None
        if X_in is not None:
            X_in = np.ascontiguousarray(np.asarray(X_in, np.float32).reshape(n, 4, 4))
            o["X_out"] = np.zeros((n, 4, 4), np.float32)
            xin, xout = _fptr(X_in), _fptr(o["X_out"])
        self._chk(self._L.symmicp_ctx_solve_probe(self._h, int(mode), int(bool(exact_rc)), S.ctypes.data_as(C.POINTER(Sums)), n, pv, xin,
                                                  o["status"].ctypes.data_as(C.POINTER(C.c_int32)), _fptr(o["pbar"]), _fptr(o["qbar"]),
                                                  _fptr(o["a"]), _fptr(o["t"]), _fptr(o["rcond"]), _fptr(o["out16"]), xout))
        return o

    def loop_solve(self, mode, sums, X_in=None, pivot=None, diff_threshold=1.0, fixed_iters=0, max_iters=10, iters=0, small_step=0,
                   eps_rotation=0.0, eps_translation=0.0, incremental=0):
        S = Sums()
        for k, v in enumerate(np.asarray(sums, np.float64).reshape(NSUM)):
            S.s[k] = v
        X_in = np.ascontiguousarray(np.eye(4, dtype=np.float32) if X_in is None else np.asarray(X_in, np.float32).reshape(16))
        pv = None if pivot is None else _fptr(np.ascontiguousarray(pivot, np.float32))
        ii = np.array([mode, fixed_iters, max_iters, iters, small_step, incremental], np.int32)
        ff = np.array([diff_threshold, eps_rotation, eps_translation], np.float32)
        st = np.zeros(4, np.int32); X = np.zeros(16, np.float32); Xa = np.zeros(12, np.float32)
        ri = np.zeros(16, np.float32); rX = np.zeros(16, np.float32); rrc = np.zeros(1, np.float32); r2 = np.zeros(2, np.int32)
        i32 = lambda a: a.ctypes.data_as(C.POINTER(C.c_int32))
        self._chk(self._L.symmicp_ctx_loop_solve(self._h, C.byref(S), pv, _fptr(X_in), i32(ii), _fptr(ff), i32(st), _fptr(X), _fptr(Xa),
                                                 _fptr(ri), _fptr(rX), _fptr(rrc), i32(r2)))
        return dict(stop=int(st[0]), reason=int(st[1]), iters=int(st[2]), small_step=int(st[3]), X=X.reshape(4, 4), Xapply=Xa.reshape(3, 4),
                    ring_increment=ri.reshape(4, 4), ring_X=rX.reshape(4, 4), ring_rcond=float(rrc[0]), ring_status=int(r2[0]), ring_solved=int(r2[1]))

    def index_info(self):
        o = IndexInfo()
        o.struct_size = C.sizeof(IndexInfo)
        self._chk(self._L.symmicp_ctx_index_info(self._h, C.byref(o)))
        d = {k: getattr(o, k) for k, _ in IndexInfo._fields_ if k != "struct_size"}
        d["origin"] = np.array(o.origin, np.float32)
        for k in ("h0", "h", "inv_h"):
            d[k] = np.float32(d[k])
        d["level_off"] = np.array(o.level_off, np.uint32)
        d["olevel_off"] = np.array(o.olevel_off, np.uint32)
        d["level_hist"] = np.array(o.level_hist, np.uint32)
        d["surface_like"] = bool(o.surface_like)
        return d

    def index_arrays(self):
        d = self.index_info()
        gl = d["grid_level"] > 0
        d["tq"] = np.zeros((d["n"], 4), np.float32)
        d["tn"] = np.zeros((d["n"], 2, 4), np.float32)
        d["boxes"] = np.zeros((d["n_boxes"], 2, 4), np.float32)
        d["ctop"] = np.zeros(d["ctop_len"] if gl else 0, np.uint32)
        d["cells"] = np.zeros(((d["n_blocks"] if gl else 0) * 512, 2), np.uint32)
        d["onodes"] = np.zeros((d["n_onodes"], 2, 4), np.float32)
        u32 = lambda a: a.ctypes.data_as(C.POINTER(C.c_uint32)) if a.size else None
        self._chk(self._L.symmicp_ctx_index_arrays(self._h, _fptr(d["tq"]), _fptr(d["tn"]), _fptr(d["boxes"]), u32(d["ctop"]), u32(d["cells"]),
                                                   _fptr(d["onodes"])))
        return d

    def source_share(self):
        nl, npk, so, ck = C.c_size_t(0), C.c_size_t(0), C.c_int32(0), C.c_int32(0)
        self._chk(self._L.symmicp_ctx_source_share(self._h, C.byref(nl), C.byref(npk), C.byref(so), C.byref(ck), None, None))
        order = np.zeros(nl.value, np.uint32) if so.value else None
        tab = np.zeros((npk.value, 2), np.uint32)
        u32 = lambda a: a.ctypes.data_as(C.POINTER(C.c_uint32)) if a is not None and a.size else None
        self._chk(self._L.symmicp_ctx_source_share(self._h, None, None, None, None, u32(order), u32(tab)))
        return dict(n_local=nl.value, pkt_count=npk.value, sorted=bool(so.value), cost_keyed=bool(ck.value), order=order, pkt_tab=tab)

    def radix_sort_probe(self, keys, vals, key_bits):
        k = np.array(keys, np.uint32).reshape(-1)
        v = np.array(vals, np.uint32).reshape(-1)
        if k.shape != v.shape:
            raise ValueError("keys and vals differ in length")
        u32 = lambda a: a.ctypes.data_as(C.POINTER(C.c_uint32))
        self._chk(self._L.symmicp_ctx_radix_sort_probe(self._h, u32(k), u32(v), k.size, int(key_bits)))
        return k, v

    def select_probe(self, keys, k):
        a = np.ascontiguousarray(np.asarray(keys, np.uint32).reshape(-1))
        kth, nle = C.c_uint32(0), C.c_uint64(0)
        self._chk(self._L.symmicp_ctx_select_probe(self._h, a.ctypes.data_as(C.POINTER(C.c_uint32)), a.size, int(k), C.byref(kth), C.byref(nle)))
        return kth.value, nle.value

    def unique_probe(self, tgt_row, d2_bits, n_t):
        r = np.ascontiguousarray(np.asarray(tgt_row, np.int32).reshape(-1))
        d = np.ascontiguousarray(np.asarray(d2_bits, np.uint32).reshape(-1))
        if r.size != d.size:
            raise ValueError("unique_probe: tgt_row and d2_bits differ in length")
        w = np.zeros(r.size, np.uint8)
        self._chk(self._L.symmicp_ctx_unique_probe(self._h, r.ctypes.data_as(C.POINTER(C.c_int32)), d.ctypes.data_as(C.POINTER(C.c_uint32)),
                                                   r.size, int(n_t), w.ctypes.data_as(C.POINTER(C.c_uint8))))
        return w.astype(bool)

    def scan_probe(self, data):
        d = np.array(data, np.uint32).reshape(-1)
        self._chk(self._L.symmicp_ctx_scan_probe(self._h, d.ctypes.data_as(C.POINTER(C.c_uint32)), d.size))
        return d

    def set_loop_log(self, on=True):
        self._chk(self._L.symmicp_set_loop_log(self._h, int(bool(on))))

    def loop_log(self):
        n = C.c_size_t(0)
        self._chk(self._L.symmicp_get_loop_log(self._h, None, 0, C.byref(n)))
        buf = (LoopLogEntry * max(1, n.value))()
        self._chk(self._L.symmicp_get_loop_log(self._h, buf, n.value, C.byref(n)))
        out = []
        for e in buf[:n.value]:
            out.append(dict(sums=np.array(e.sums[:], np.float64), increment=np.array(e.increment[:], np.float32).reshape(4, 4),
                            X=np.array(e.X[:], np.float32).reshape(4, 4), rcond=e.rcond, iter=e.iter, status=e.status, solved=e.solved,
                            list_len=e.list_len, reason=e.reason, batch=e.batch))
        return out


class MyICP:

    def __init__(self, mode=MODE_QUIRKS, corr=CORR_IDENTITY, max_iters=10, diff_threshold=1.0, verbose=True, **extra):
        self._cfg = dict(mode=mode, corr=corr, max_iters=max_iters, diff_threshold=diff_threshold,
                         verbose=int(bool(verbose)), **extra)
        self.cloud_src = self.cloud_tgt = None
        self.normals_src = self.normals_tgt = None
        self._final = np.eye(4, dtype=np.float32)
        self.last_result = None
        self._loss = (LOSS_NONE, 0.0)
        self._gicp_eps = None
        self._trim = 1.0
        self._one_to_one = False
        self._median = 0.0
        self._color_weight = None
        self.intensity_src = self.intensity_tgt = None
        self._levels = []
        self.level_results = []
        self._global = None
        self.global_result = None
        self._have_src = self._have_tgt = False

    def setMaxCorrespondenceDistance(self, d):
        self._cfg["max_corr_dist"] = float(d)

    def setVoxelLevels(self, levels):
# ... 187 lines not shown
```

### include/symmicp.h

```cpp
#ifndef SYMMICP_H
#define SYMMICP_H

#include <stddef.h>
#include <stdint.h>

#ifdef __cplusplus
extern "C" {
#endif

#define SYMMICP_NSUM 40
#define SYMMICP_UNIQUE_ID_BYTES 128

typedef enum {
    SYMMICP_OK = 0,
    SYMMICP_ERR_ARG = 1,
    SYMMICP_ERR_SIZE = 2,
    SYMMICP_ERR_DEGENERATE = 3,
    SYMMICP_ERR_IO = 4,
    SYMMICP_ERR_HIP = 5,
    SYMMICP_ERR_STATE = 6,
    SYMMICP_ERR_COMM = 7,
    SYMMICP_ERR_NO_CONSENSUS = 8
} symmicp_status;

// ... 60 lines not shown
int symmicp_get_robust_loss(const symmicp_ctx *ctx, int *loss, float *scale);
int symmicp_set_gicp_epsilon(symmicp_ctx *ctx, float eps);
int symmicp_get_gicp_epsilon(const symmicp_ctx *ctx, float *eps);
int symmicp_set_color_weight(symmicp_ctx *ctx, float lambda);
int symmicp_get_color_weight(const symmicp_ctx *ctx, float *lambda);
int symmicp_set_trim_fraction(symmicp_ctx *ctx, float fraction);
int symmicp_get_trim_fraction(const symmicp_ctx *ctx, float *fraction);
int symmicp_get_trim_state(const symmicp_ctx *ctx, uint64_t *candidates, uint64_t *kept, float *tau_d2);
int symmicp_set_one_to_one(symmicp_ctx *ctx, int on);
int symmicp_get_one_to_one(const symmicp_ctx *ctx, int *on);
int symmicp_set_median_factor(symmicp_ctx *ctx, float factor);
int symmicp_get_median_factor(const symmicp_ctx *ctx, float *factor);
int symmicp_get_rejection_state(const symmicp_ctx *ctx, uint64_t *gated, uint64_t *unique, uint64_t *kept, float *tau_d2);
float symmicp_robust_weight(int loss, float scale, float r);

int symmicp_set_source(symmicp_ctx *ctx, const float *xyz, size_t xyz_row_stride, size_t xyz_col_stride,
                       const float *nrm, size_t nrm_row_stride, size_t nrm_col_stride, size_t n);
int symmicp_set_target(symmicp_ctx *ctx, const float *xyz, size_t xyz_row_stride, size_t xyz_col_stride,
                       const float *nrm, size_t nrm_row_stride, size_t nrm_col_stride, size_t n);

int symmicp_set_source_intensity(symmicp_ctx *ctx, const float *intensity, size_t stride, size_t n);
int symmicp_set_target_intensity(symmicp_ctx *ctx, const float *intensity, size_t stride,
                                 const float *grad, size_t grad_row_stride, size_t grad_col_stride, size_t n);
int symmicp_get_source_intensity(symmicp_ctx *ctx, float *intensity, size_t cap);

int symmicp_align(symmicp_ctx *ctx, const float *guess16, symmicp_result *out);
int symmicp_begin(symmicp_ctx *ctx, const float *guess16, symmicp_iter_result *out);
int symmicp_step(symmicp_ctx *ctx, symmicp_iter_result *out);
int symmicp_get_transform(const symmicp_ctx *ctx, float out16[16]);
size_t symmicp_format_result(const float transform16[16], char *buf, size_t cap);
int symmicp_get_pivot(const symmicp_ctx *ctx, float out3[3]);
int symmicp_get_correspondences(symmicp_ctx *ctx, int32_t *idx, float *d2, size_t cap);
int symmicp_get_source(symmicp_ctx *ctx, float *xyz, float *nrm, size_t cap);
int symmicp_get_certificates(symmicp_ctx *ctx, float *cert4, uint32_t *hood8, float *hood_radius, int32_t *winner_row, size_t cap);
size_t symmicp_local_source_count(const symmicp_ctx *ctx);
size_t symmicp_local_source_offset(const symmicp_ctx *ctx);

int symmicp_solve(int mode, const symmicp_sums *sums, const float pivot[3],
                  float pbar[3], float qbar[3], float a[3], float t[3], float *rcond, float out16[16]);

int symmicp_ctx_solve_probe(symmicp_ctx *ctx, int mode, int exact_rc, const symmicp_sums *sums, size_t n, const float pivot[3],
                            const float *X_in16, int32_t *status, float *pbar, float *qbar, float *a, float *t, float *rcond,
                            float *out16, float *X_out16);
int symmicp_ctx_loop_solve(symmicp_ctx *ctx, const symmicp_sums *sums, const float pivot[3], const float X_in16[16], const int32_t in_i[6],
                           const float in_f[3], int32_t state_out[4], float X_out16[16], float Xapply_out12[12], float ring_inc16[16],
                           float ring_X16[16], float *ring_rcond, int32_t ring_i2[2]);
typedef struct {
    double sums[SYMMICP_NSUM];
    float increment[16], X[16];
    float rcond;
    int32_t iter;
    int32_t status;
    int32_t solved;
    int32_t list_len;
    int32_t reason;
    int32_t batch;
    int32_t reserved;
} symmicp_loop_log_entry;
int symmicp_set_loop_log(symmicp_ctx *ctx, int on);
int symmicp_get_loop_log(const symmicp_ctx *ctx, symmicp_loop_log_entry *out, size_t cap, size_t *count);

typedef struct {
    int32_t struct_size;
    uint32_t n;
    int32_t grid_level;
    int32_t gdim;
    float origin[3];
    float h0, h, inv_h;
    int32_t tree_levels;
    int32_t top;
    uint32_t ntop;
    uint32_t level_off[12];
    uint32_t n_boxes;
    uint32_t olevel_off[12];
    uint32_t n_onodes;
    uint32_t n_blocks;
    uint32_t ctop_len;
    uint32_t leaf_max;
    int32_t surface_like;
    uint32_t level_hist[16];
} symmicp_index_info;
int symmicp_ctx_index_info(symmicp_ctx *ctx, symmicp_index_info *info);
int symmicp_ctx_index_arrays(symmicp_ctx *ctx, float *tq, float *tn, float *boxes, uint32_t *ctop, uint32_t *cells, float *onodes);
int symmicp_ctx_source_share(symmicp_ctx *ctx, size_t *n_local, size_t *pkt_count, int32_t *sorted, int32_t *cost_keyed, uint32_t *order,
                             uint32_t *pkt_tab);
int symmicp_ctx_radix_sort_probe(symmicp_ctx *ctx, uint32_t *keys, uint32_t *vals, size_t n, int key_bits);
int symmicp_ctx_scan_probe(symmicp_ctx *ctx, uint32_t *data, size_t n);
int symmicp_ctx_select_probe(symmicp_ctx *ctx, const uint32_t *keys, size_t n, uint64_t k, uint32_t *kth_out, uint64_t *n_le_out);
int symmicp_ctx_unique_probe(symmicp_ctx *ctx, const int32_t *tgt_row, const uint32_t *d2_bits, size_t n, size_t n_t, uint8_t *winner_out);

int symmicp_estimate_normals(int device, const float *xyz, size_t row_stride, size_t col_stride, size_t n, int k,
                             const float viewpoint[3], float *nrm_out, float *curv_out);
int symmicp_ctx_estimate_normals(symmicp_ctx *ctx, const float *xyz, size_t row_stride, size_t col_stride, size_t n, int k,
                                 const float viewpoint[3], float *nrm_out, float *curv_out);
int symmicp_ctx_knn(symmicp_ctx *ctx, const float *xyz, size_t row_stride, size_t col_stride, size_t n, int k,
                    int32_t *rows_out, float *d2_out);

int symmicp_ctx_intensity_gradient(symmicp_ctx *ctx, const float *xyz, size_t xyz_row_stride, size_t xyz_col_stride,
                                   const float *nrm, size_t nrm_row_stride, size_t nrm_col_stride,
                                   const float *intensity, size_t intensity_stride, size_t n, int k, float *grad_out);
int symmicp_intensity_gradient(int device, const float *xyz, size_t xyz_row_stride, size_t xyz_col_stride,
                               const float *nrm, size_t nrm_row_stride, size_t nrm_col_stride,
                               const float *intensity, size_t intensity_stride, size_t n, int k, float *grad_out);

int symmicp_ctx_radius_search(symmicp_ctx *ctx, const float *xyz, size_t row_stride, size_t col_stride, size_t n, float radius,
                              int32_t *count_out, int64_t *offsets_out, int32_t *rows_out, float *d2_out, size_t cap,
                              size_t *total_out);
int symmicp_radius_search(int device, const float *xyz, size_t row_stride, size_t col_stride, size_t n, float radius,
                          int32_t *count_out, int64_t *offsets_out, int32_t *rows_out, float *d2_out, size_t cap, size_t *total_out);

int symmicp_ctx_fpfh(symmicp_ctx *ctx, const float *xyz, size_t xyz_row_stride, size_t xyz_col_stride,
                     const float *nrm, size_t nrm_row_stride, size_t nrm_col_stride, size_t n, float radius,
                     float *fpfh_out, float *spfh_out, int32_t *count_out);
int symmicp_fpfh(int device, const float *xyz, size_t xyz_row_stride, size_t xyz_col_stride,
                 const float *nrm, size_t nrm_row_stride, size_t nrm_col_stride, size_t n, float radius,
                 float *fpfh_out, float *spfh_out, int32_t *count_out);

int symmicp_ctx_feature_nn(symmicp_ctx *ctx, const float *fa, size_t na, const float *fb, size_t nb,
                           int32_t *nn_out, float *d2_out, float *d2_second_out);
int symmicp_feature_nn(int device, const float *fa, size_t na, const float *fb, size_t nb,
                       int32_t *nn_out, float *d2_out, float *d2_second_out);
int symmicp_ctx_feature_correspondences(symmicp_ctx *ctx, const float *fa, size_t na, const float *fb, size_t nb, int mutual,
                                        float max_ratio, int32_t *pairs_out, float *d2_out, size_t cap, size_t *count_out);
int symmicp_feature_correspondences(int device, const float *fa, size_t na, const float *fb, size_t nb, int mutual,
                                    float max_ratio, int32_t *pairs_out, float *d2_out, size_t cap, size_t *count_out);

typedef struct {
    uint32_t struct_size;
    uint32_t hypotheses;
    uint64_t seed;
    float max_dist;
    float edge_ratio;
    int32_t refits;
    int32_t reserved;
} symmicp_ransac_config;
typedef struct {
    int32_t best_hypothesis;
    int32_t evaluated;
    int32_t inliers_ransac;
    int32_t inliers_final;
    double rmse_final;
    double transform[16];
} symmicp_ransac_result;
#define SYMMICP_RANSAC_EVALUATED 0
#define SYMMICP_RANSAC_REPEATED 1
#define SYMMICP_RANSAC_EDGE 2
#define SYMMICP_RANSAC_DEGENERATE 3
#define SYMMICP_RANSAC_FAR 4
void symmicp_ransac_config_default(symmicp_ransac_config *cfg);
int symmicp_ctx_ransac(symmicp_ctx *ctx, const float *src_xyz, size_t src_row_stride, size_t src_col_stride, size_t ns,
                       const float *tgt_xyz, size_t tgt_row_stride, size_t tgt_col_stride, size_t nt,
                       const int32_t *pairs, size_t m, const symmicp_ransac_config *cfg, float transform16[16],
                       symmicp_ransac_result *result, uint8_t *inlier_mask_out, uint8_t *status_out, int32_t *inliers_out);
int symmicp_ransac(int device, const float *src_xyz, size_t src_row_stride, size_t src_col_stride, size_t ns,
                   const float *tgt_xyz, size_t tgt_row_stride, size_t tgt_col_stride, size_t nt,
                   const int32_t *pairs, size_t m, const symmicp_ransac_config *cfg, float transform16[16],
                   symmicp_ransac_result *result, uint8_t *inlier_mask_out, uint8_t *status_out, int32_t *inliers_out);
int symmicp_ctx_ransac_hypotheses(symmicp_ctx *ctx, const float *src_xyz, size_t src_row_stride, size_t src_col_stride, size_t ns,
                                  const float *tgt_xyz, size_t tgt_row_stride, size_t tgt_col_stride, size_t nt,
                                  const int32_t *pairs, size_t m, const symmicp_ransac_config *cfg, float *hyp_out,
                                  uint8_t *status_out, float pivots_out[6]);

int symmicp_ctx_voxel_downsample(symmicp_ctx *ctx, const float *xyz, size_t xyz_row_stride, size_t xyz_col_stride,
                                 const float *nrm, size_t nrm_row_stride, size_t nrm_col_stride, size_t n, float leaf, int min_points,
                                 float *xyz_out, float *nrm_out, int32_t *count_out, int32_t *voxel_of, size_t cap, size_t *n_out);
int symmicp_voxel_downsample(int device, const float *xyz, size_t xyz_row_stride, size_t xyz_col_stride,
// ... 41 lines not shown
```

Measured before the change: 30550.

## Add finer second-level cell grid and per-block occupancy bitmaps to pass scan

Builds a second, finer Morton cell table (picked by a fine points-per-cell target) alongside the coarse grid, plus 64-bit occupancy bitmaps per 8x8 row slab so the pass kernel can skip empty cells in a 27-cell neighbourhood without reading cell ranges. The per-point scan now runs on the fine grid and adds a coarse fallback round for points whose fine search cannot certify. The goal is to shrink candidate-cell scans and wasted memory reads in the nearest-neighbour correspondence pass. In exchange it costs extra index build time and memory, an extra kernel round, and more branching and register pressure in the hot kernel.

```diff
diff --git a/icp-symm_amd/csrc/engine.cpp b/icp-symm_amd/csrc/engine.cpp
--- a/icp-symm_amd/csrc/engine.cpp
+++ b/icp-symm_amd/csrc/engine.cpp
@@ -14,6 +14,8 @@
     if (const char *e = std::getenv("SYMMICP_GRID_PPC")) w.grid_ppc = std::atof(e);
     w.grid_maxlevel = (int)num("SYMMICP_GRID_MAXLEVEL", kMortonBits);
     w.grid_level = (int)num("SYMMICP_GRID_LEVEL", -1);
+    if (const char *e = std::getenv("SYMMICP_FINE_PPC")) w.fine_ppc = std::atof(e);
+    w.no_cell_bitmap = flag("SYMMICP_NO_CELL_BITMAP");
     if (const char *e = std::getenv("SYMMICP_FIRST_PASS")) w.first_pass = (e[0] == 'p') ? 1 : 0;
     w.oct_leaf = (int)num("SYMMICP_OCT_LEAF", 0);
     if (const char *e = std::getenv("SYMMICP_PACKET_ORDER")) w.packet_order = e[0] != '0';
@@ -597,7 +599,7 @@
     launch_gather_f4(cl.x, cl.y, cl.z, cl.nx, cl.ny, cl.nz, order.p, n, tq, tn, c->stream);
     TargetIndex ix{};
     ix.tq = tq; ix.tn = tn; ix.n = n;
-    int glevel = 0;
+    int glevel = 0, fine_level = 0;
     if (want_grid) {
         DevBuf<uint32_t> hist;
         HIP_TRY(c, hist.alloc_temp(c->arena, 16));
@@ -618,6 +620,13 @@
         if (c->sw.grid_level >= 0) glevel = c->sw.grid_level;
         if (glevel > lcap) glevel = lcap;
         if (glevel < 0) glevel = 0;
+        if (c->sw.fine_ppc > 0.0) {
+            double o = 1.0;
+            for (int l = 1; l <= lcap; l++) {
+                o += (double)hh[l];
+                if ((double)n / o >= c->sw.fine_ppc) fine_level = l;
+            }
+        }
         {
             double occ_l[kMortonBits + 1];
             double o = 1.0;
@@ -630,8 +639,8 @@
         }
     }
     ix.glevel = glevel;
-    if (glevel > 0) {
-        const int ltop = glevel > 3 ? glevel - 3 : 0;
+    auto build_table = [&](int level, uint32_t **ctop_p, uint2 **cells_p, unsigned long long **occ_p, uint32_t *nblocks_p, uint32_t *ntop_p) -> int {
+        const int ltop = level > 3 ? level - 3 : 0;
         const size_t ntop = (size_t)1 << (3 * ltop);
         DevBuf<uint32_t> nid_top, scan_ws;
         HIP_TRY(c, nid_top.alloc_temp(c->arena, n));
@@ -645,19 +654,43 @@
         const int tshift = 3 * (kMortonBits - ltop);
         const bool last_starts = (n == 1) || (tshift < 30 && (kl[1] >> tshift) != (kl[0] >> tshift));
         const size_t nblocks = (size_t)last_excl + (last_starts ? 1 : 0);
-        if (notes) { notes->nblocks = (uint32_t)nblocks; notes->ctop_len = (uint32_t)ntop; }
-        HIP_TRY(c, keep_alloc(c, (void **)ctop_out, sizeof(uint32_t) * ntop));
-        HIP_TRY(c, hipMemsetAsync(*ctop_out, 0xFF, sizeof(uint32_t) * ntop, c->stream));
-        HIP_TRY(c, keep_alloc(c, (void **)cells_out, sizeof(uint2) * nblocks * 512));
-        HIP_TRY(c, hipMemsetAsync(*cells_out, 0, sizeof(uint2) * nblocks * 512, c->stream));
-        launch_cell_table(keys.p, n, glevel, nid_top.p, *ctop_out, *cells_out, c->stream);
+        *nblocks_p = (uint32_t)nblocks; *ntop_p = (uint32_t)ntop;
+        HIP_TRY(c, keep_alloc(c, (void **)ctop_p, sizeof(uint32_t) * ntop));
+        HIP_TRY(c, hipMemsetAsync(*ctop_p, 0xFF, sizeof(uint32_t) * ntop, c->stream));
+        HIP_TRY(c, keep_alloc(c, (void **)cells_p, sizeof(uint2) * nblocks * 512));
+        HIP_TRY(c, hipMemsetAsync(*cells_p, 0, sizeof(uint2) * nblocks * 512, c->stream));
+        launch_cell_table(keys.p, n, level, nid_top.p, *ctop_p, *cells_p, c->stream);
+        if (occ_p) {
+            HIP_TRY(c, keep_alloc(c, (void **)occ_p, sizeof(unsigned long long) * nblocks * 8));
+            launch_cell_occupancy(*cells_p, (uint32_t)nblocks, *occ_p, c->stream);
+        }
         HIP_TRY(c, hipStreamSynchronize(c->stream));
+        return SYMMICP_OK;
+    };
+    if (glevel > 0) {
+        const bool want_occ = ctop_out && !c->sw.no_cell_bitmap;
+        unsigned long long *occ = nullptr;
+        uint32_t nblocks = 0, ntop = 0;
+        st = build_table(glevel, ctop_out, cells_out, want_occ ? &occ : nullptr, &nblocks, &ntop);
+        if (st != SYMMICP_OK) return st;
+        if (notes) { notes->nblocks = nblocks; notes->ctop_len = ntop; }
         ix.ctop = *ctop_out;
         ix.cells = *cells_out;
+        ix.occ = occ;
         ix.gdim = 1 << glevel;
         ix.ox = origin[0]; ix.oy = origin[1]; ix.oz = origin[2];
         ix.h = h0 * (float)(1 << (kMortonBits - glevel));
         ix.inv_h = (1.0f / h0) / (float)(1 << (kMortonBits - glevel));
+        int flevel = 0;
+        if (ctop_out && fine_level > glevel) flevel = fine_level;
+        if (flevel) {
+            uint32_t *ctop_f = nullptr; uint2 *cells_f = nullptr; unsigned long long *occ_f = nullptr;
+            uint32_t nblocks_f = 0, ntop_f = 0;
+            st = build_table(flevel, &ctop_f, &cells_f, want_occ ? &occ_f : nullptr, &nblocks_f, &ntop_f);
+            if (st != SYMMICP_OK) return st;
+            ix.ctop_f = ctop_f; ix.cells_f = cells_f; ix.occ_f = occ_f; ix.fshift = flevel - glevel;
+            if (notes) { notes->nblocks_f = nblocks_f; notes->ctop_len_f = ntop_f; }
+        }
     }
     uint32_t cnt[kMaxTreeLevels], pad[kMaxTreeLevels];
     int nl = 0;
@@ -714,7 +747,7 @@
             else (void)hipGetLastError();
         }
     }
-    arena_begin(c->arena, n * (96 + 4 * (xr + nr)) + ((size_t)1 << 20));
+    arena_begin(c->arena, n * (104 + 4 * (xr + nr)) + ((size_t)1 << 20));
     double cen[3];
     DevBuf<float> tblock;
     int st = upload_planar(c, xyz, xr, xc, nrm, nr, nc, n, tblock, false, cen);
diff --git a/icp-symm_amd/csrc/engine_debug.cpp b/icp-symm_amd/csrc/engine_debug.cpp
--- a/icp-symm_amd/csrc/engine_debug.cpp
+++ b/icp-symm_amd/csrc/engine_debug.cpp
@@ -22,6 +22,6 @@
             std::fprintf(stderr, "[symmicp dbg] pass %lld (packets): steps=%llu nodes+leaf candidates=%llu leaf candidates rejected=%llu points=%llu tie rescans=%llu overflows=%llu lanes wanting a scanned leaf (sum)=%llu | packet ticks (10 ns): sum=%llu max=%llu\n",
                          (long long)c->st.passes, h[0], h[4], h[5], h[3], h[2], h[1], h[8], h[7], h[6]);
         else
-        std::fprintf(stderr, "[symmicp dbg] pass %lld: cells: certified=%llu (by neighbourhood %llu) scans=%llu (neighbourhoods kept %llu, not kept %llu) probes=%llu to-walk=%llu items=%llu points=%llu | walk list=%lld visits=%llu wave-max*64=%llu\n",
-                     (long long)c->st.passes, h[1], h[8], h[2], h[9], h[10], h[6], h[7], h[0], h[3], list_len, h[4], h[5]);
+        std::fprintf(stderr, "[symmicp dbg] pass %lld: cells: certified=%llu (by neighbourhood %llu) scans=%llu (neighbourhoods kept %llu, not kept %llu) probes=%llu to-walk=%llu items=%llu points=%llu coarse rounds=%llu | walk list=%lld visits=%llu wave-max*64=%llu\n",
+                     (long long)c->st.passes, h[1], h[8], h[2], h[9], h[10], h[6], h[7], h[0], h[3], h[11], list_len, h[4], h[5]);
 }
diff --git a/icp-symm_amd/csrc/engine_internal.h b/icp-symm_amd/csrc/engine_internal.h
--- a/icp-symm_amd/csrc/engine_internal.h
+++ b/icp-symm_amd/csrc/engine_internal.h
@@ -72,6 +72,8 @@
     std::string debug_trace;
     double grid_ppc = 3.0;
     int grid_maxlevel = kMortonBits, grid_level = -1;
+    double fine_ppc = 2.0;
+    bool no_cell_bitmap = false;
     int first_pass = -1;
     int oct_leaf = 0;
     bool packet_order = true;
@@ -113,6 +115,7 @@
     uint32_t hist[16] = {};
     uint32_t leaf_max = 0;
     uint32_t nblocks = 0, ctop_len = 0;
+    uint32_t nblocks_f = 0, ctop_len_f = 0;
 };
 
 struct symmicp_ctx {
diff --git a/icp-symm_amd/csrc/engine_probe.cpp b/icp-symm_amd/csrc/engine_probe.cpp
--- a/icp-symm_amd/csrc/engine_probe.cpp
+++ b/icp-symm_amd/csrc/engine_probe.cpp
@@ -76,6 +76,42 @@
     return SYMMICP_OK;
 }
 
+int symmicp_ctx_fine_cells(symmicp_ctx *c, int32_t *fine_level, uint32_t *n_blocks_f, uint32_t *ctop_len_f, int32_t *have_occ,
+                           uint32_t *ctop_f, uint32_t *cells_f, uint64_t *occ_f, uint64_t *occ)
+{
+    if (!c) return SYMMICP_ERR_ARG;
+    if (!has_target_index(c)) return fail(c, SYMMICP_ERR_STATE, "fine_cells: no target index (SYMMICP_CORR_TREE after set_target)");
+    const TargetIndex &ix = c->ix;
+    const bool fine = ix.fshift > 0;
+    const size_t nbf = fine ? c->notes.nblocks_f : 0, ntf = fine ? c->notes.ctop_len_f : 0, nb = ix.glevel > 0 ? c->notes.nblocks : 0;
+    if (fine_level) *fine_level = fine ? ix.glevel + ix.fshift : 0;
+    if (n_blocks_f) *n_blocks_f = (uint32_t)nbf;
+    if (ctop_len_f) *ctop_len_f = (uint32_t)ntf;
+    if (have_occ) *have_occ = ix.occ ? 1 : 0;
+    HIP_TRY(c, hipSetDevice(c->device));
+    const struct { void *dst; const void *src; size_t bytes; } parts[] = {
+        {ctop_f, ix.ctop_f, sizeof(uint32_t) * ntf},
+        {cells_f, ix.cells_f, sizeof(uint2) * 512 * nbf},
+        {occ_f, ix.occ_f, ix.occ_f ? sizeof(uint64_t) * 8 * nbf : 0},
+        {occ, ix.occ, ix.occ ? sizeof(uint64_t) * 8 * nb : 0},
+    };
+    for (const auto &p : parts) {
+        const int st = copy_back(c, p.dst, p.src, p.bytes);
+        if (st != SYMMICP_OK) { (void)hipStreamSynchronize(c->stream); return st; }
+    }
+    HIP_TRY(c, hipStreamSynchronize(c->stream));
+    return SYMMICP_OK;
+}
+
+int symmicp_ctx_pass_search(symmicp_ctx *c, int64_t *searched, int64_t *list_len)
+{
+    if (!c) return SYMMICP_ERR_ARG;
+    if (c->cfg.corr != SYMMICP_CORR_TREE) return fail(c, SYMMICP_ERR_STATE, "pass_search: not a SYMMICP_CORR_TREE context");
+    if (searched) *searched = (int64_t)c->last_uncertified;
+    if (list_len) *list_len = (int64_t)c->last_list_len;
+    return SYMMICP_OK;
+}
+
 int symmicp_ctx_source_share(symmicp_ctx *c, size_t *n_local, size_t *pkt_count, int32_t *sorted, int32_t *cost_keyed, uint32_t *order,
                              uint32_t *pkt_tab)
 {
diff --git a/icp-symm_amd/csrc/kernels_build.hip b/icp-symm_amd/csrc/kernels_build.hip
--- a/icp-symm_amd/csrc/kernels_build.hip
+++ b/icp-symm_amd/csrc/kernels_build.hip
@@ -276,6 +276,18 @@
     if (i == n - 1 || (keys[i + 1] >> shift) != c) slot->y = i + 1;
 }
 
+__global__ __launch_bounds__(256) void k_cell_occupancy(const uint2 *__restrict__ cells, uint32_t nblocks, unsigned long long *occ)
+{
+    const uint32_t g = blockIdx.x * blockDim.x + threadIdx.x;
+    const uint32_t blk = g >> 9, z = (g >> 6) & 7u, y = (g >> 3) & 7u, x = g & 7u;
+    if (blk >= nblocks) return;
+    const uint32_t m = (x & 1u) | ((y & 1u) << 1) | ((z & 1u) << 2) | ((x & 2u) << 2) | ((y & 2u) << 3) | ((z & 2u) << 4) |
+                       ((x & 4u) << 4) | ((y & 4u) << 5) | ((z & 4u) << 6);
+    const uint2 r = cells[(size_t)blk * 512u + m];
+    const unsigned long long w = __ballot(r.y > r.x);
+    if ((threadIdx.x & 63u) == 0) occ[(size_t)blk * 8u + z] = w;
+}
+
 __global__ __launch_bounds__(256) void k_leaf_boxes(const float4 *__restrict__ tq, uint32_t n, float4 *boxes, uint32_t nleaf_padded)
 {
     uint32_t l = blockIdx.x * blockDim.x + threadIdx.x;
@@ -498,6 +510,11 @@
     hipLaunchKernelGGL(k_cell_table, dim3(nblk(n, 256)), dim3(256), 0, s, keys, n, shift, 3 * (kMortonBits - ltop), nid_top, ctop, cells);
 }
 
+void launch_cell_occupancy(const uint2 *cells, uint32_t nblocks, unsigned long long *occ, hipStream_t s)
+{
+    if (nblocks) hipLaunchKernelGGL(k_cell_occupancy, dim3(nblocks * 2u), dim3(256), 0, s, cells, nblocks, occ);
+}
+
 void launch_leaf_boxes(const float4 *tq, uint32_t n, float4 *boxes, uint32_t nleaf_padded, hipStream_t s)
 {
     hipLaunchKernelGGL(k_leaf_boxes, dim3(nblk(nleaf_padded, 256)), dim3(256), 0, s, tq, n, boxes, nleaf_padded);
diff --git a/icp-symm_amd/csrc/kernels_pass.hip b/icp-symm_amd/csrc/kernels_pass.hip
--- a/icp-symm_amd/csrc/kernels_pass.hip
+++ b/icp-symm_amd/csrc/kernels_pass.hip
@@ -404,11 +404,11 @@
     acc_block_reduce_store(acc, a.partials, blockIdx.x);
 }
 
-__device__ __forceinline__ uint2 cell_range(const TargetIndex &ix, uint32_t morton)
-{
-    const uint32_t blk = ix.ctop[morton >> 9];
+__device__ __forceinline__ uint2 cell_range(const uint32_t *__restrict__ ctop, const uint2 *__restrict__ cells, uint32_t morton)
+{
+    const uint32_t blk = ctop[morton >> 9];
     if (blk == 0xFFFFFFFFu) return make_uint2(0u, 0u);
-    return ix.cells[(size_t)blk * 512u + (morton & 511u)];
+    return cells[(size_t)blk * 512u + (morton & 511u)];
 }
 
 __device__ __forceinline__ uint32_t spread3(uint32_t v)
@@ -482,6 +482,57 @@
         a.cert[i].w = cert_word(0.0f, true);
     }
     return true;
+}
+
+struct CellGrid {
+    const uint32_t *ctop;
+    const uint2 *cells;
+    const unsigned long long *occ;
+    int gdim;
+    float h, inv_h;
+};
+__device__ __forceinline__ CellGrid scan_grid(const TargetIndex &ix)
+{
+    CellGrid g;
+    const bool fine = ix.fshift > 0;
+    const float s = (float)(1 << ix.fshift);
+    g.ctop = fine ? ix.ctop_f : ix.ctop; g.cells = fine ? ix.cells_f : ix.cells; g.occ = fine ? ix.occ_f : ix.occ;
+    g.gdim = ix.gdim << ix.fshift; g.h = ix.h / s; g.inv_h = ix.inv_h * s;
+    return g;
+}
+
+__device__ __forceinline__ uint32_t cells_occ27(const uint32_t *__restrict__ ctop, const unsigned long long *__restrict__ occ, int gdim, int x0, int y0, int z0)
+{
+    const int xs = x0 >> 3, ys = y0 >> 3;
+    const bool twox = (min(x0 + 2, gdim - 1) >> 3) != xs, twoy = (min(y0 + 2, gdim - 1) >> 3) != ys;
+    const uint32_t mx0 = spread3((uint32_t)xs), mx1 = spread3((uint32_t)xs + 1u), my0 = spread3((uint32_t)ys) << 1, my1 = spread3((uint32_t)ys + 1u) << 1;
+    uint32_t b00 = 0xFFFFFFFFu, b01 = 0xFFFFFFFFu, b10 = 0xFFFFFFFFu, b11 = 0xFFFFFFFFu;
+    int zs = -1;
+    uint32_t out = 0;
+#pragma unroll 1
+    for (int kz = 0; kz < 3; kz++) {
+        const int z = min(z0 + kz, gdim - 1);
+        if ((z >> 3) != zs) {
+            zs = z >> 3;
+            const uint32_t mz = spread3((uint32_t)zs) << 2;
+            b00 = ctop[mz | my0 | mx0];
+            b01 = twox ? ctop[mz | my0 | mx1] : 0xFFFFFFFFu;
+            b10 = twoy ? ctop[mz | my1 | mx0] : 0xFFFFFFFFu;
+            b11 = (twox && twoy) ? ctop[mz | my1 | mx1] : 0xFFFFFFFFu;
+        }
+        const uint32_t zw = (uint32_t)z & 7u;
+        const unsigned long long w00 = b00 != 0xFFFFFFFFu ? occ[(size_t)b00 * 8u + zw] : 0ull, w01 = b01 != 0xFFFFFFFFu ? occ[(size_t)b01 * 8u + zw] : 0ull;
+        const unsigned long long w10 = b10 != 0xFFFFFFFFu ? occ[(size_t)b10 * 8u + zw] : 0ull, w11 = b11 != 0xFFFFFFFFu ? occ[(size_t)b11 * 8u + zw] : 0ull;
+#pragma unroll
+        for (int ky = 0; ky < 3; ky++) {
+            const int y = y0 + ky;
+            const bool up = (y >> 3) != ys;
+            const int sh = (y & 7) * 8;
+            const uint32_t row = ((uint32_t)((up ? w10 : w00) >> sh) & 0xFFu) | (((uint32_t)((up ? w11 : w01) >> sh) & 0xFFu) << 8);
+            out |= ((row >> (x0 & 7)) & 7u) << (3 * ky + 9 * kz);
+        }
+    }
+    return out;
 }
 
 template <bool HOOD>
@@ -506,6 +557,8 @@
     const bool active = i < a.n;
     const float inf = __int_as_float(0x7f800000);
     const uint32_t push_shard = from_list ? ((i / kPassThreads) & (uint32_t)(kShards - 1)) : shard;
+    const CellGrid g = scan_grid(ix);
+    const bool fine = ix.fshift > 0;
 
     float px = 0.f, py = 0.f, pz = 0.f;
     Best b;
@@ -513,6 +566,9 @@
     uint32_t mask = 0;
     uint32_t mask_rest = 0;
     bool defer = false, searched = false, probe = false, uncert = false, hood_ok = false;
+    bool coarse = false;
+    int pstage = 0;
+    int bx0 = 0, by0 = 0, bz0 = 0;
     float lim = 0.f, lim_full = 0.f;
     float reach = 0.f;
     if (active) {
@@ -542,14 +598,14 @@
             uncert = true;
             defer = true;
             if (b.pos >= 0 && ix.glevel > 0) {
-                const float margin = 2e-3f * ix.h;
-                const float gmax = (float)ix.gdim;
+                const float margin = 2e-3f * g.h;
+                const float gmax = (float)g.gdim;
                 const float rb = __builtin_amdgcn_sqrtf(b.d2) * 1.00001f;
-                lim = rb + kSlackFrac * ix.h;
+                lim = rb + kSlackFrac * g.h;
                 const float r = lim + margin;
-                const float lx = (px - r - ix.ox) * ix.inv_h, hx = (px + r - ix.ox) * ix.inv_h;
-                const float ly = (py - r - ix.oy) * ix.inv_h, hy = (py + r - ix.oy) * ix.inv_h;
-                const float lz = (pz - r - ix.oz) * ix.inv_h, hz = (pz + r - ix.oz) * ix.inv_h;
+                const float lx = (px - r - ix.ox) * g.inv_h, hx = (px + r - ix.ox) * g.inv_h;
+                const float ly = (py - r - ix.oy) * g.inv_h, hy = (py + r - ix.oy) * g.inv_h;
+                const float lz = (pz - r - ix.oz) * g.inv_h, hz = (pz + r - ix.oz) * g.inv_h;
                 const int x0 = (int)floorf(fminf(fmaxf(lx, 0.0f), gmax - 1.0f)), x1 = (int)floorf(fminf(fmaxf(hx, 0.0f), gmax - 1.0f));
                 const int y0 = (int)floorf(fminf(fmaxf(ly, 0.0f), gmax - 1.0f)), y1 = (int)floorf(fminf(fmaxf(hy, 0.0f), gmax - 1.0f));
                 const int z0 = (int)floorf(fminf(fmaxf(lz, 0.0f), gmax - 1.0f)), z1 = (int)floorf(fminf(fmaxf(hz, 0.0f), gmax - 1.0f));
@@ -561,9 +617,9 @@
                     float gx[3], gy[3], gz[3];
 #pragma unroll
                     for (int k = 0; k < 3; k++) {
-                        gx[k] = (k <= nx) ? axis_gap2(px, ix.ox, x0 + k, ix.h, margin) : inf;
-                        gy[k] = (k <= ny) ? axis_gap2(py, ix.oy, y0 + k, ix.h, margin) : inf;
-                        gz[k] = (k <= nz) ? axis_gap2(pz, ix.oz, z0 + k, ix.h, margin) : inf;
+                        gx[k] = (k <= nx) ? axis_gap2(px, ix.ox, x0 + k, g.h, margin) : inf;
+                        gy[k] = (k <= ny) ? axis_gap2(py, ix.oy, y0 + k, g.h, margin) : inf;
+                        gz[k] = (k <= nz) ? axis_gap2(pz, ix.oz, z0 + k, g.h, margin) : inf;
                     }
 #pragma unroll
                     for (int kz = 0; kz < 3; kz++)
@@ -575,19 +631,20 @@
                                 if (g2 <= thr2) mask |= 1u << (kx + 3 * ky + 9 * kz);
                             }
                     s_cell0[tid] = (uint32_t)x0 | ((uint32_t)y0 << 10) | ((uint32_t)z0 << 20);
+                    bx0 = x0; by0 = y0; bz0 = z0;
                     reach = rb;
                 }
             }
             if (defer && b.pos >= 0 && ix.glevel > 0) {
-                const float fx = (px - ix.ox) * ix.inv_h, fy = (py - ix.oy) * ix.inv_h, fz = (pz - ix.oz) * ix.inv_h;
-                const float gmax = (float)ix.gdim;
+                const float fx = (px - ix.ox) * g.inv_h, fy = (py - ix.oy) * g.inv_h, fz = (pz - ix.oz) * g.inv_h;
+                const float gmax = (float)g.gdim;
                 if (fx >= 0.0f && fy >= 0.0f && fz >= 0.0f && fx < gmax && fy < gmax && fz < gmax) {
                     const int cx = (int)fx, cy = (int)fy, cz = (int)fz;
                     const int x0 = max(cx - 1, 0), y0 = max(cy - 1, 0), z0 = max(cz - 1, 0);
-                    const int x1 = min(cx + 1, ix.gdim - 1), y1 = min(cy + 1, ix.gdim - 1), z1 = min(cz + 1, ix.gdim - 1);
-                    const int ax = max(cx - ((fx - (float)cx) < 0.5f ? 1 : 0), 0), bx = min(ax + 1, ix.gdim - 1);
-                    const int ay = max(cy - ((fy - (float)cy) < 0.5f ? 1 : 0), 0), by = min(ay + 1, ix.gdim - 1);
-                    const int az = max(cz - ((fz - (float)cz) < 0.5f ? 1 : 0), 0), bz = min(az + 1, ix.gdim - 1);
+                    const int x1 = min(cx + 1, g.gdim - 1), y1 = min(cy + 1, g.gdim - 1), z1 = min(cz + 1, g.gdim - 1);
+                    const int ax = max(cx - ((fx - (float)cx) < 0.5f ? 1 : 0), 0), bx = min(ax + 1, g.gdim - 1);
+                    const int ay = max(cy - ((fy - (float)cy) < 0.5f ? 1 : 0), 0), by = min(ay + 1, g.gdim - 1);
+                    const int az = max(cz - ((fz - (float)cz) < 0.5f ? 1 : 0), 0), bz = min(az + 1, g.gdim - 1);
 #pragma unroll
                     for (int kz = 0; kz < 3; kz++)
 #pragma unroll
@@ -602,25 +659,31 @@
                                 }
                             }
                     s_cell0[tid] = (uint32_t)x0 | ((uint32_t)y0 << 10) | ((uint32_t)z0 << 20);
+                    bx0 = x0; by0 = y0; bz0 = z0;
                     float face = inf, face8 = inf;
-                    if (x0 > 0) face = fminf(face, px - (ix.ox + (float)x0 * ix.h));
-                    if (y0 > 0) face = fminf(face, py - (ix.oy + (float)y0 * ix.h));
-                    if (z0 > 0) face = fminf(face, pz - (ix.oz + (float)z0 * ix.h));
-                    if (x1 < ix.gdim - 1) face = fminf(face, (ix.ox + (float)(x1 + 1) * ix.h) - px);
-                    if (y1 < ix.gdim - 1) face = fminf(face, (ix.oy + (float)(y1 + 1) * ix.h) - py);
-                    if (z1 < ix.gdim - 1) face = fminf(face, (ix.oz + (float)(z1 + 1) * ix.h) - pz);
-                    if (ax > 0) face8 = fminf(face8, px - (ix.ox + (float)ax * ix.h));
-                    if (ay > 0) face8 = fminf(face8, py - (ix.oy + (float)ay * ix.h));
-                    if (az > 0) face8 = fminf(face8, pz - (ix.oz + (float)az * ix.h));
-                    if (bx < ix.gdim - 1) face8 = fminf(face8, (ix.ox + (float)(bx + 1) * ix.h) - px);
-                    if (by < ix.gdim - 1) face8 = fminf(face8, (ix.oy + (float)(by + 1) * ix.h) - py);
-                    if (bz < ix.gdim - 1) face8 = fminf(face8, (ix.oz + (float)(bz + 1) * ix.h) - pz);
-                    lim = face8 - 2e-3f * ix.h;
-                    lim_full = face - 2e-3f * ix.h;
+                    if (x0 > 0) face = fminf(face, px - (ix.ox + (float)x0 * g.h));
+                    if (y0 > 0) face = fminf(face, py - (ix.oy + (float)y0 * g.h));
+                    if (z0 > 0) face = fminf(face, pz - (ix.oz + (float)z0 * g.h));
+                    if (x1 < g.gdim - 1) face = fminf(face, (ix.ox + (float)(x1 + 1) * g.h) - px);
+                    if (y1 < g.gdim - 1) face = fminf(face, (ix.oy + (float)(y1 + 1) * g.h) - py);
+                    if (z1 < g.gdim - 1) face = fminf(face, (ix.oz + (float)(z1 + 1) * g.h) - pz);
+                    if (ax > 0) face8 = fminf(face8, px - (ix.ox + (float)ax * g.h));
+                    if (ay > 0) face8 = fminf(face8, py - (ix.oy + (float)ay * g.h));
+                    if (az > 0) face8 = fminf(face8, pz - (ix.oz + (float)az * g.h));
+                    if (bx < g.gdim - 1) face8 = fminf(face8, (ix.ox + (float)(bx + 1) * g.h) - px);
+                    if (by < g.gdim - 1) face8 = fminf(face8, (ix.oy + (float)(by + 1) * g.h) - py);
+                    if (bz < g.gdim - 1) face8 = fminf(face8, (ix.oz + (float)(bz + 1) * g.h) - pz);
+                    lim = face8 - 2e-3f * g.h;
+                    lim_full = face - 2e-3f * g.h;
                     probe = true;
+                    pstage = 1;
                     defer = false;
                     reach = __builtin_amdgcn_sqrtf(b.d2) * 1.00001f;
                 }
+            }
+            if (g.occ && (mask | mask_rest)) {
+                const uint32_t o = cells_occ27(g.ctop, g.occ, g.gdim, bx0, by0, bz0);
+                mask &= o; mask_rest &= o;
             }
             if (defer) {
                 a.pos_out[i] = b.pos;
@@ -645,7 +708,7 @@
     } else reach = 0.0f;
     if (HOOD) { s_reach[tid] = reach; s_hcnt[tid] = 0; s_qi[tid] = i; }
     uint32_t total = 0, total_all = 0;
-    for (int round = 0; round < 2; round++) {
+    for (int round = 0; round < 3; round++) {
     const uint32_t cnt = (uint32_t)__popc(mask);
     uint32_t incl = cnt;
 #pragma unroll
@@ -738,8 +801,9 @@
             const int bit = (int)(item & 31u);
             const int kz = bit / 9, ky = (bit - 9 * kz) / 3, kx = bit - 9 * kz - 3 * ky;
             const uint32_t c0 = s_cell0[q];
-            const uint32_t cx = (c0 & 1023u) + (uint32_t)kx, cy = ((c0 >> 10) & 1023u) + (uint32_t)ky, cz = (c0 >> 20) + (uint32_t)kz;
-            const uint2 rng = cell_range(ix, (spread3(cz) << 2) | (spread3(cy) << 1) | spread3(cx));
+            const uint32_t cx = (c0 & 1023u) + (uint32_t)kx, cy = ((c0 >> 10) & 1023u) + (uint32_t)ky, cz = ((c0 >> 20) & 1023u) + (uint32_t)kz;
+            const bool crs = (c0 >> 30) != 0u;
+            const uint2 rng = cell_range(crs ? ix.ctop : g.ctop, crs ? ix.cells : g.cells, (spread3(cz) << 2) | (spread3(cy) << 1) | spread3(cx));
             if (ix.dbg) atomicAdd(ix.dbg + 3, (unsigned long long)(rng.y - rng.x));
             j0 = rng.x; j1 = rng.y;
             while (j1 > j0 && j1 - j0 > kItemMax) {
@@ -765,15 +829,57 @@
     }
     __syncthreads();
 
-    bool more = false;
-    if (round == 0 && probe) {
-        const float d1 = sqrtf(__uint_as_float((uint32_t)(s_key[tid] >> 32))) * 1.00001f;
-        if (!(d1 * 1.02f < lim)) { more = (mask_rest != 0); lim = lim_full; }
-    }
-    mask = more ? mask_rest : 0u;
-    if (round == 1) break;
+    mask = 0u;
+    if (pstage) {
+        const float dsq = sqrtf(__uint_as_float((uint32_t)(s_key[tid] >> 32)));
+        const float d1 = dsq * 1.00001f;
+        if (pstage == 1) {
+            if (d1 * 1.02f < lim) pstage = 0;
+            else { lim = lim_full; mask = mask_rest; pstage = 2; }
+        }
+        if (pstage == 2 && !mask) {
+            pstage = 0;
+            if (fine && !(dsq * 1.000001f < lim)) {
+                float qx = px, qy = py, qz = pz;
+                asm volatile("" : "+v"(qx), "+v"(qy), "+v"(qz));
+                const float hc = ix.h, mc = 2e-3f * ix.h;
+                const int gm = ix.gdim - 1;
+                const int cx = min((int)((qx - ix.ox) * ix.inv_h), gm), cy = min((int)((qy - ix.oy) * ix.inv_h), gm), cz = min((int)((qz - ix.oz) * ix.inv_h), gm);
+                const int x0 = max(cx - 1, 0), y0 = max(cy - 1, 0), z0 = max(cz - 1, 0);
+                const int x1 = min(cx + 1, gm), y1 = min(cy + 1, gm), z1 = min(cz + 1, gm);
+                const float thr2 = d1 * d1;
+#pragma unroll 1
+                for (int kz = 0; kz < 3; kz++) {
+                    const float gzk = (z0 + kz <= z1) ? axis_gap2(qz, ix.oz, z0 + kz, hc, mc) : inf;
+#pragma unroll 1
+                    for (int ky = 0; ky < 3; ky++) {
+                        const float gyz = ((y0 + ky <= y1) ? axis_gap2(qy, ix.oy, y0 + ky, hc, mc) : inf) + gzk;
+#pragma unroll 1
+                        for (int kx = 0; kx < 3; kx++) {
+                            const float gxk = (x0 + kx <= x1) ? axis_gap2(qx, ix.ox, x0 + kx, hc, mc) : inf;
+                            if (gxk + gyz <= thr2) mask |= 1u << (kx + 3 * ky + 9 * kz);
+                        }
+                    }
+                }
+                s_cell0[tid] = (uint32_t)x0 | ((uint32_t)y0 << 10) | ((uint32_t)z0 << 20) | (1u << 30);
+                float face = inf;
+                if (x0 > 0) face = fminf(face, qx - (ix.ox + (float)x0 * hc));
+                if (y0 > 0) face = fminf(face, qy - (ix.oy + (float)y0 * hc));
+                if (z0 > 0) face = fminf(face, qz - (ix.oz + (float)z0 * hc));
+                if (x1 < gm) face = fminf(face, (ix.ox + (float)(x1 + 1) * hc) - qx);
+                if (y1 < gm) face = fminf(face, (ix.oy + (float)(y1 + 1) * hc) - qy);
+                if (z1 < gm) face = fminf(face, (ix.oz + (float)(z1 + 1) * hc) - qz);
+                lim = face - mc;
+                coarse = true;
+                if (HOOD) s_reach[tid] = 0.0f;
+                if (mask) pstage = 3;
+                if (ix.dbg) atomicAdd(ix.dbg + 11, 1ull);
+            }
+        } else if (pstage == 3) pstage = 0;
+    }
+    if (round == (fine ? 2 : 1)) break;
     {
-        const unsigned long long anym = __ballot(more);
+        const unsigned long long anym = __ballot(mask != 0u);
         if (lane == 0) s_anyw[wave] = (anym != 0ull);
         __syncthreads();
         uint32_t any = 0;
@@ -803,6 +909,9 @@
             a.cert[i].w = 0.0f;
             a.pairrec[2 * (size_t)i + 1].w = 2.0f;
             sl_push(wl.work, push_shard, i);
+        } else if (coarse) {
+            a.cert[i] = make_float4(px, py, pz, 0.0f);
+            store_pair_record(a, ix, i, s_pos[tid]);
         } else {
             const float second = sqrtf(__uint_as_float(s_second[tid])) * 0.999999f;
             const float L = fminf(second, lim * 0.99999f);
diff --git a/icp-symm_amd/csrc/symmicp_internal.h b/icp-symm_amd/csrc/symmicp_internal.h
--- a/icp-symm_amd/csrc/symmicp_internal.h
+++ b/icp-symm_amd/csrc/symmicp_internal.h
@@ -58,6 +58,10 @@
     unsigned long long *dbg_trace;
     const float4 *onodes;
     uint32_t olevel_off[kMortonBits + 2];
+    const unsigned long long *occ, *occ_f;
+    const uint32_t *ctop_f;
+    const uint2 *cells_f;
+    int32_t fshift;
 };
 
 constexpr uint32_t kOctCfMask = 0x0FFFFFFFu;
@@ -197,6 +201,7 @@
 void launch_deinterleave3(const float *raw, size_t row_stride, size_t offset, uint32_t n, float *x, float *y, float *z, hipStream_t s);
 void launch_level_hist(const uint32_t *keys, uint32_t n, uint32_t *hist16, hipStream_t s);
 void launch_cell_table(const uint32_t *keys, uint32_t n, int glevel, const uint32_t *nid_top, uint32_t *ctop, uint2 *cells, hipStream_t s);
+void launch_cell_occupancy(const uint2 *cells, uint32_t nblocks, unsigned long long *occ , hipStream_t s);
 void launch_oct_flags(const uint32_t *keys, uint32_t n, int level, uint32_t *nid, hipStream_t s);
 void launch_exclusive_scan(uint32_t *data, uint32_t n, uint32_t *tile_ws , hipStream_t s);
 void launch_oct_first(const uint32_t *keys, uint32_t n, int level, const uint32_t *nid, uint32_t *first, hipStream_t s);
diff --git a/icp-symm_amd/py/symmicp/__init__.py b/icp-symm_amd/py/symmicp/__init__.py
--- a/icp-symm_amd/py/symmicp/__init__.py
+++ b/icp-symm_amd/py/symmicp/__init__.py
@@ -105,6 +105,7 @@
     "symmicp_feature_nn", "symmicp_ctx_feature_nn", "symmicp_feature_correspondences", "symmicp_ctx_feature_correspondences",
     "symmicp_ransac_config_default", "symmicp_ransac", "symmicp_ctx_ransac", "symmicp_ctx_ransac_hypotheses",
     "symmicp_ctx_index_info", "symmicp_ctx_index_arrays", "symmicp_ctx_source_share", "symmicp_ctx_radix_sort_probe", "symmicp_ctx_scan_probe",
+    "symmicp_ctx_fine_cells", "symmicp_ctx_pass_search",
     "symmicp_set_trim_fraction", "symmicp_get_trim_fraction", "symmicp_get_trim_state", "symmicp_ctx_select_probe",
     "symmicp_set_one_to_one", "symmicp_get_one_to_one", "symmicp_set_median_factor", "symmicp_get_median_factor",
     "symmicp_get_rejection_state", "symmicp_ctx_unique_probe",
@@ -209,6 +210,9 @@
     u32p, szp = C.POINTER(C.c_uint32), C.POINTER(C.c_size_t)
     L.symmicp_ctx_index_info.argtypes = [vp, C.POINTER(IndexInfo)]
     L.symmicp_ctx_index_arrays.argtypes = [vp, fp, fp, fp, u32p, u32p, fp]
+    L.symmicp_ctx_pass_search.argtypes = [vp, C.POINTER(C.c_int64), C.POINTER(C.c_int64)]
+    L.symmicp_ctx_fine_cells.argtypes = [vp, C.POINTER(C.c_int32), C.POINTER(C.c_uint32), C.POINTER(C.c_uint32), C.POINTER(C.c_int32), u32p, u32p,
+                                         C.POINTER(C.c_uint64), C.POINTER(C.c_uint64)]
     L.symmicp_ctx_source_share.argtypes = [vp, szp, szp, i32p, i32p, u32p, u32p]
     L.symmicp_ctx_radix_sort_probe.argtypes = [vp, u32p, u32p, C.c_size_t, C.c_int]
     L.symmicp_ctx_scan_probe.argtypes = [vp, u32p, C.c_size_t]
@@ -963,6 +967,23 @@
         u32 = lambda a: a.ctypes.data_as(C.POINTER(C.c_uint32)) if a.size else None
         self._chk(self._L.symmicp_ctx_index_arrays(self._h, _fptr(d["tq"]), _fptr(d["tn"]), _fptr(d["boxes"]), u32(d["ctop"]), u32(d["cells"]),
                                                    _fptr(d["onodes"])))
+        return d
+
+    def pass_search(self):
+        a, b = C.c_int64(0), C.c_int64(0)
+        self._chk(self._L.symmicp_ctx_pass_search(self._h, C.byref(a), C.byref(b)))
+        return a.value, b.value
+
+    def fine_cells(self):
+        fl, nbf, ntf, ho = C.c_int32(0), C.c_uint32(0), C.c_uint32(0), C.c_int32(0)
+        self._chk(self._L.symmicp_ctx_fine_cells(self._h, C.byref(fl), C.byref(nbf), C.byref(ntf), C.byref(ho), None, None, None, None))
+        info = self.index_info()
+        nb = info["n_blocks"] if info["grid_level"] > 0 else 0
+        d = dict(fine_level=fl.value, have_occ=bool(ho.value), ctop_f=np.zeros(ntf.value, np.uint32), cells_f=np.zeros((nbf.value * 512, 2), np.uint32),
+                 occ_f=np.zeros((nbf.value if ho.value else 0, 8), np.uint64), occ=np.zeros((nb if ho.value else 0, 8), np.uint64))
+        u32 = lambda a: a.ctypes.data_as(C.POINTER(C.c_uint32)) if a.size else None
+        u64 = lambda a: a.ctypes.data_as(C.POINTER(C.c_uint64)) if a.size else None
+        self._chk(self._L.symmicp_ctx_fine_cells(self._h, None, None, None, None, u32(d["ctop_f"]), u32(d["cells_f"]), u64(d["occ_f"]), u64(d["occ"])))
         return d
 
     def source_share(self):
diff --git a/include/symmicp.h b/include/symmicp.h
--- a/include/symmicp.h
+++ b/include/symmicp.h
@@ -166,6 +166,9 @@
 } symmicp_index_info;
 int symmicp_ctx_index_info(symmicp_ctx *ctx, symmicp_index_info *info);
 int symmicp_ctx_index_arrays(symmicp_ctx *ctx, float *tq, float *tn, float *boxes, uint32_t *ctop, uint32_t *cells, float *onodes);
+int symmicp_ctx_fine_cells(symmicp_ctx *ctx, int32_t *fine_level, uint32_t *n_blocks_f, uint32_t *ctop_len_f, int32_t *have_occ,
+                           uint32_t *ctop_f, uint32_t *cells_f, uint64_t *occ_f, uint64_t *occ);
+int symmicp_ctx_pass_search(symmicp_ctx *ctx, int64_t *searched, int64_t *list_len);
 int symmicp_ctx_source_share(symmicp_ctx *ctx, size_t *n_local, size_t *pkt_count, int32_t *sorted, int32_t *cost_keyed, uint32_t *order,
                              uint32_t *pkt_tab);
 int symmicp_ctx_radix_sort_probe(symmicp_ctx *ctx, uint32_t *keys, uint32_t *vals, size_t n, int key_bits);
```

Result: slower. 18180 (-40.5%).
